# Jiawei-Yang/Denoising-ViT

Measured on AMD Instinct MI355X. Metric: stage-1 images denoised/sec (DINOv2-B/14, 518px, 1k Adam steps), higher is better.
Workload: dtype bf16

## Files before the change

denoising-vit_amd/csrc/dvt_fit_fused.hip:

```cpp
#include "dvt_common.h"
#include "dvt_grid_dev.h"
#include "dvt_loss_row.h"

typedef short bf16x8 __attribute__((ext_vector_type(8)));
typedef float f32x4 __attribute__((ext_vector_type(4)));

int g_fit_rows32 = 1;
int g_fit_xcd_affinity = 1;
int g_fit_small_wg = 0;

namespace {

constexpr int FR0 = 16;
constexpr int FW8 = 8;
constexpr int FE = 128;

template <bool F32>
struct Op {
  static constexpr int ES = F32 ? 4 : 2;
  static constexpr int KS = F32 ? 16 : 32;
};
typedef unsigned u32x4f __attribute__((ext_vector_type(4)));

template <bool F32>
__host__ __device__ constexpr int apitch(int K) { return K * Op<F32>::ES + 16; }

struct FusedArgs {
  DvtGridTable T;
  DvtShadowLayout S;
  DvtTLayout TL;
  int n, lattice;
  int xcd_group;
  float grad_scale;
  long long off_grid, off_b1, off_b2, off_G, off_bh1, off_bh2, off_bh3;
  DvtFusedFit f[DVT_FIT_BATCH_MAX];
};

__device__ __forceinline__ uint16_t bf16_of(float v) { return (uint16_t)(dvt_pack_bf16x2(v, 0.f) & 0xffffu); }

template <int NC, int FR, int FW, bool F32>
__device__ __forceinline__ void store_T(const char* img, void* __restrict__ dstTv, int B, int b0, int tid) {
  constexpr int RPP = F32 ? 4 : 8;
  for (int item = tid; item < NC * (FR / RPP); item += 64 * FW) {
    const int grp = item / NC, col = item - grp * NC;
    const int brow = b0 + grp * RPP;
    const char* src = img + grp * RPP * apitch<F32>(NC) + col * Op<F32>::ES;
    if constexpr (F32) {
      const int sg = brow >> 4, g = (brow >> 2) & 3;
      float4 v;
      v.x = *reinterpret_cast<const float*>(src);
      v.y = *reinterpret_cast<const float*>(src + apitch<F32>(NC));
      v.z = *reinterpret_cast<const float*>(src + 2 * apitch<F32>(NC));
      v.w = *reinterpret_cast<const float*>(src + 3 * apitch<F32>(NC));
      const long long off = ((long long)(col >> 4) * (B >> 4) + sg) * 256 + (((g << 4) + (col & 15)) << 2);
      *reinterpret_cast<float4*>(static_cast<float*>(dstTv) + off) = v;
    } else {
      const int kstep = brow >> 5, g = (brow >> 3) & 3;
      uint32_t w[4];
#pragma unroll
      for (int j = 0; j < 4; ++j) {
        const uint32_t lo = *reinterpret_cast<const uint16_t*>(src + (2 * j) * apitch<F32>(NC));
        const uint32_t hi = *reinterpret_cast<const uint16_t*>(src + (2 * j + 1) * apitch<F32>(NC));
        w[j] = lo | (hi << 16);
      }
      const long long off = ((long long)(col >> 4) * (B >> 5) + kstep) * 512 + (((g << 4) + (col & 15)) << 3);
      *reinterpret_cast<uint4*>(static_cast<uint16_t*>(dstTv) + off) = make_uint4(w[0], w[1], w[2], w[3]);
    }
  }
}

template <int K, int N, bool RELU, bool MASK, int RB, int FW, bool F32>
__device__ __forceinline__ void mlp_layer(const char* actA, const void* __restrict__ Wv,
                                          const float* __restrict__ bias, char* act_out,
                                          float* __restrict__ gout, const char* mask, int wave, int lane) {
  constexpr int KS = Op<F32>::KS, ES = Op<F32>::ES;
  constexpr int NTILES = N / 16, NT = (NTILES + FW - 1) / FW, S = K / KS;
  constexpr int INFL = FW == 8 ? 24 : 16;
  constexpr int PD0 = INFL / NT > 16 ? 16 : (INFL / NT < 1 ? 1 : INFL / NT);
  constexpr int PD = PD0 < S ? PD0 : S;
  static_assert(K % KS == 0 && N % 16 == 0, "layer shape");
  const int lc = lane & 15, g = lane >> 4;
  f32x4 acc[RB][NT];
  const char* wp[NT];
#pragma unroll
  for (int i = 0; i < NT; ++i) {
#pragma unroll
    for (int rb = 0; rb < RB; ++rb) acc[rb][i] = (f32x4){0.f, 0.f, 0.f, 0.f};
    const int t = wave + FW * i;
    const int tt = (NTILES % FW == 0 || t < NTILES) ? t : 0;
    wp[i] = static_cast<const char*>(Wv) + (size_t)tt * S * 1024 + lane * 16;
  }
  u32x4f b[PD][NT];
#pragma unroll
  for (int p = 0; p < PD; ++p)
#pragma unroll
    for (int i = 0; i < NT; ++i) b[p][i] = *reinterpret_cast<const u32x4f*>(wp[i] + 1024 * p);
  __builtin_amdgcn_sched_barrier(0);
  const char* ap = actA + lc * apitch<F32>(K) + g * 16;
#pragma unroll
  for (int s = 0; s < S; ++s) {
    u32x4f av[RB];
#pragma unroll
    for (int rb = 0; rb < RB; ++rb) av[rb] = *reinterpret_cast<const u32x4f*>(ap + rb * 16 * apitch<F32>(K) + s * 64);
    if constexpr (F32) {
#pragma unroll
      for (int j = 0; j < 4; ++j)
#pragma unroll
        for (int i = 0; i < NT; ++i)
#pragma unroll
          for (int rb = 0; rb < RB; ++rb)
            acc[rb][i] = __builtin_amdgcn_mfma_f32_16x16x4f32(__uint_as_float(av[rb][j]), __uint_as_float(b[s % PD][i][j]),
                                                              acc[rb][i], 0, 0, 0);
    } else {
#pragma unroll
      for (int i = 0; i < NT; ++i)
#pragma unroll
        for (int rb = 0; rb < RB; ++rb)
          acc[rb][i] = __builtin_amdgcn_mfma_f32_16x16x32_bf16(__builtin_bit_cast(bf16x8, av[rb]),
                                                               __builtin_bit_cast(bf16x8, b[s % PD][i]), acc[rb][i], 0, 0, 0);
    }
    if (s + PD < S) {
#pragma unroll
      for (int i = 0; i < NT; ++i) b[s % PD][i] = *reinterpret_cast<const u32x4f*>(wp[i] + 1024 * (s + PD));
    }
    __builtin_amdgcn_sched_barrier(0);
  }
#pragma unroll
  for (int i = 0; i < NT; ++i) {
    const int t = wave + FW * i;
    if (NTILES % FW != 0 && t >= NTILES) continue;
    const int n = t * 16 + lc;
    const float bv = bias != nullptr ? bias[n] : 0.f;
#pragma unroll
    for (int rb = 0; rb < RB; ++rb)
#pragma unroll
      for (int r = 0; r < 4; ++r) {
        const int row = rb * 16 + 4 * g + r;
        float v = acc[rb][i][r] + bv;
        if (RELU) v = fmaxf(v, 0.f);
        if (MASK) {
          if constexpr (F32) {
            v = *reinterpret_cast<const float*>(mask + row * apitch<F32>(N) + n * ES) > 0.f ? v : 0.f;
          } else {
            const uint16_t m = *reinterpret_cast<const uint16_t*>(mask + row * apitch<F32>(N) + n * ES);
            v = (m != 0 && !(m & 0x8000u)) ? v : 0.f;
          }
        }
        if (act_out != nullptr) {
          if constexpr (F32) *reinterpret_cast<float*>(act_out + row * apitch<F32>(N) + n * ES) = v;
          else *reinterpret_cast<uint16_t*>(act_out + row * apitch<F32>(N) + n * ES) = bf16_of(v);
        }
        if (gout != nullptr) gout[(size_t)row * N + n] = v;
      }
  }
}

template <int C, bool PH2, int FR, bool F32 = false>
struct FusedLds {
  static constexpr int H = C / 2, R = C / 4;
  static constexpr int O_ENC = 0;
  static constexpr int O_H1 = O_ENC + FR * apitch<F32>(FE);
  static constexpr int O_DF = O_H1 + FR * apitch<F32>(H);
  static constexpr int O_RAW = O_DF + FR * apitch<F32>(C);
  static constexpr int O_R1 = O_RAW + FR * apitch<F32>(C);
  static constexpr int O_R2 = O_R1 + FR * apitch<F32>(R);
  static constexpr int TOTAL = PH2 ? O_R2 + FR * apitch<F32>(R) : O_RAW;
};
template <int C>
constexpr bool fused_f32_fits() { return FusedLds<C, true, 16, true>::TOTAL <= 160 * 1024; }

template <int C, bool PH2, int FR, int FW, bool F32 = false>
__global__ __launch_bounds__(64 * FW) void fit_rows_kernel(FusedArgs a) {
  using L = FusedLds<C, PH2, FR, F32>;
  constexpr int RB = FR / 16;
  constexpr int ES = Op<F32>::ES;
  static_assert(FR == 16 || FR == 32, "rows per workgroup");
  static_assert(FW == 8 || (FW == 4 && FR == 16), "waves per workgroup");
  static_assert(!F32 || (FR == 16 && FW == 8), "fp32 operands: 16 rows, 8 waves");
  static_assert(L::TOTAL <= 160 * 1024, "LDS images of the row kernel");
  constexpr int H = C / 2, R = C / 4, E = FE, cq = C / 4;
  __shared__ __attribute__((aligned(16))) char smem[L::TOTAL];
  int fit_, rb_;
  if (a.xcd_group > 0) {
    const int lin = (int)blockIdx.x + (int)blockIdx.y * (int)gridDim.x, xcd = lin & 7, j = lin >> 3;
    fit_ = xcd / a.xcd_group;
    rb_ = j * a.xcd_group + xcd % a.xcd_group;
  } else {
    fit_ = (int)blockIdx.y;
    rb_ = (int)blockIdx.x;
  }
  const DvtFusedFit& f = a.f[fit_];
  const int tid = threadIdx.x, lane = tid & 63;
  const int wave = __builtin_amdgcn_readfirstlane(tid >> 6);
  const int row0 = rb_ * FR;
  const char* __restrict__ sh = static_cast<const char*>(f.shadow);
  const float* __restrict__ P = f.params;
  const float4* __restrict__ feat4 = reinterpret_cast<const float4*>(f.feat);

  uint32_t warm[5] = {0u, 0u, 0u, 0u, 0u};
  {
    constexpr int LPR = (C * 4 + 127) / 128;
    const int j = lane % 32;
#pragma unroll
    for (int rr = lane / 32; rr < FR / FW; rr += 2) {
      if (j < LPR) {
        const int ri = f.ridx[row0 + wave + FW * rr];
        warm[4] ^= __float_as_uint(f.feat[(size_t)ri * C + j * 32]) ^
                   __float_as_uint(P[a.off_G + (size_t)(ri % a.lattice) * C + j * 32]);
      }
    }
  }
  {
    const int per_xcd = a.xcd_group > 0 ? (int)gridDim.x / a.xcd_group : ((int)gridDim.x + 7) / 8;
    const int nslot = per_xcd >= 16 ? 16 : per_xcd;
    const int slot = (a.xcd_group > 0 ? rb_ / a.xcd_group : (rb_ >> 3)) % nslot;
    const long long lines = ((PH2 ? a.S.total : a.S.direct[2]) * ES + 127) / 128;
    const long long per = (lines + nslot - 1) / nslot;
    const long long l0 = slot * per, l1 = l0 + per < lines ? l0 + per : lines;
    const uint32_t* w32 = reinterpret_cast<const uint32_t*>(sh);
#pragma unroll
    for (int j = 0; j < 4 * RB * (8 / FW); ++j) {
      const long long li = l0 + tid + (long long)j * 64 * FW;
      if (li < l1) warm[j & 3] ^= w32[li * 32];
    }
  }

  if (tid < FR * 16) {
    const int r = tid >> 4, l = tid & 15;
    const float2 p = reinterpret_cast<const float2*>(f.xy)[f.ridx[row0 + r]];
    uint32_t idx[4];
    float w[4];
    corners2d(a.T, l, p.x, p.y, idx, w);
    const float4* __restrict__ grid = reinterpret_cast<const float4*>(P + a.off_grid);
    float4 lo = make_float4(0.f, 0.f, 0.f, 0.f), hi = lo;
#pragma unroll
    for (int c = 0; c < 4; ++c) {
      const float4 u = grid[(size_t)idx[c] * 2], v = grid[(size_t)idx[c] * 2 + 1];
      lo.x = fmaf(w[c], u.x, lo.x);
      lo.y = fmaf(w[c], u.y, lo.y);
      lo.z = fmaf(w[c], u.z, lo.z);
      lo.w = fmaf(w[c], u.w, lo.w);
      hi.x = fmaf(w[c], v.x, hi.x);
      hi.y = fmaf(w[c], v.y, hi.y);
      hi.z = fmaf(w[c], v.z, hi.z);
      hi.w = fmaf(w[c], v.w, hi.w);
    }
    if constexpr (F32) {
      *reinterpret_cast<float4*>(smem + L::O_ENC + r * apitch<F32>(E) + l * 32) = lo;
      *reinterpret_cast<float4*>(smem + L::O_ENC + r * apitch<F32>(E) + l * 32 + 16) = hi;
    } else {
      *reinterpret_cast<uint4*>(smem + L::O_ENC + r * apitch<F32>(E) + l * 16) =
          make_uint4(dvt_pack_bf16x2(lo.x, lo.y), dvt_pack_bf16x2(lo.z, lo.w), dvt_pack_bf16x2(hi.x, hi.y),
                     dvt_pack_bf16x2(hi.z, hi.w));
    }
  }
  if (PH2) {
    for (int i = tid; i < FR * cq; i += 64 * FW) {
      const int r = i / cq, q = i - r * cq;
      const float4 v = feat4[(size_t)f.ridx[row0 + r] * cq + q];
      if constexpr (F32)
        *reinterpret_cast<float4*>(smem + L::O_RAW + r * apitch<F32>(C) + q * 16) = v;
      else
        *reinterpret_cast<uint2*>(smem + L::O_RAW + r * apitch<F32>(C) + q * 8) =
            make_uint2(dvt_pack_bf16x2(v.x, v.y), dvt_pack_bf16x2(v.z, v.w));
    }
  }
  __syncthreads();

  const int B = a.n;
  char* __restrict__ T = static_cast<char*>(f.T);
#define SH(off) (sh + (size_t)(off) * ES)
#define TT(idx) (T + (size_t)a.TL.off[idx] * ES)
  mlp_layer<E, H, true, false, RB, FW, F32>(smem + L::O_ENC, SH(a.S.direct[0]), P + a.off_b1, smem + L::O_H1, nullptr,
                               nullptr, wave, lane);
  if (PH2)
    mlp_layer<C, R, true, false, RB, FW, F32>(smem + L::O_RAW, SH(a.S.direct[2]), P + a.off_bh1, smem + L::O_R1, nullptr,
                                 nullptr, wave, lane);
  __syncthreads();
  mlp_layer<H, C, false, false, RB, FW, F32>(smem + L::O_H1, SH(a.S.direct[1]), P + a.off_b2, nullptr,
                                f.F + (size_t)row0 * C, nullptr, wave, lane);
  store_T<H, FR, FW, F32>(smem + L::O_H1, TT(DVT_T_H1), B, row0, tid);
  store_T<E, FR, FW, F32>(smem + L::O_ENC, TT(DVT_T_ENC), B, row0, tid);
  if (PH2) {
    mlp_layer<R, R, true, false, RB, FW, F32>(smem + L::O_R1, SH(a.S.direct[3]), P + a.off_bh2, smem + L::O_R2, nullptr,
                                 nullptr, wave, lane);
    store_T<C, FR, FW, F32>(smem + L::O_RAW, TT(DVT_T_RAW), B, row0, tid);
    store_T<R, FR, FW, F32>(smem + L::O_R1, TT(DVT_T_R1), B, row0, tid);
    __syncthreads();
    mlp_layer<R, C, false, false, RB, FW, F32>(smem + L::O_R2, SH(a.S.direct[4]), P + a.off_bh3, nullptr,
                                  f.Hres + (size_t)row0 * C, nullptr, wave, lane);
    store_T<R, FR, FW, F32>(smem + L::O_R2, TT(DVT_T_R2), B, row0, tid);
  }
  __syncthreads();

  static_assert(C <= 1024, "row warm-up above assumes <= 32 lines per row");
  {
    constexpr int NR = FR / FW;
    constexpr int NB = (C <= 768 && !(FW == 4 && PH2)) ? 2 : 1;
    DvtLossRowRegs<PH2> lr[NB];
#pragma unroll
    for (int r0 = 0; r0 < NR; r0 += NB) {
#pragma unroll
    for (int rr = r0; rr < r0 + NB; ++rr) {
      const int gr = row0 + wave + FW * rr;
      const int ri = f.ridx[gr];
      dvt_loss_row_load<PH2>(lr[rr - r0], reinterpret_cast<const float4*>(f.F) + (size_t)gr * cq,
                             reinterpret_cast<const float4*>(P + a.off_G) + (size_t)(ri % a.lattice) * cq,
                             PH2 ? reinterpret_cast<const float4*>(f.Hres) + (size_t)gr * cq : nullptr,
                             feat4 + (size_t)ri * cq, cq, lane);
    }
#pragma unroll
    for (int rr = r0; rr < r0 + NB; ++rr) {
      const int row = wave + FW * rr, gr = row0 + row;
      char* const img_p = smem + L::O_DF + row * apitch<F32>(C);
      char* const img_h = PH2 ? smem + L::O_RAW + row * apitch<F32>(C) : nullptr;
      dvt_loss_row_compute<PH2>(lr[rr - r0], reinterpret_cast<float4*>(f.dF) + (size_t)gr * cq,
                                nullptr, nullptr,
                                f.rows + (size_t)gr * 8, a.n, cq, a.grad_scale, lane,
                                F32 ? nullptr : reinterpret_cast<uint2*>(img_p), F32 ? nullptr : reinterpret_cast<uint2*>(img_h),
                                F32 ? reinterpret_cast<float4*>(img_p) : nullptr, F32 ? reinterpret_cast<float4*>(img_h) : nullptr);
    }
    }
  }
  __syncthreads();

  mlp_layer<C, H, false, true, RB, FW, F32>(smem + L::O_DF, SH(a.S.transp[1]), nullptr, smem + L::O_H1, nullptr,
                               smem + L::O_H1, wave, lane);
  store_T<C, FR, FW, F32>(smem + L::O_DF, TT(DVT_T_DF), B, row0, tid);
  if (PH2) {
    mlp_layer<C, R, false, true, RB, FW, F32>(smem + L::O_RAW, SH(a.S.transp[4]), nullptr, smem + L::O_R2, nullptr,
                                 smem + L::O_R2, wave, lane);
    store_T<C, FR, FW, F32>(smem + L::O_RAW, TT(DVT_T_DH), B, row0, tid);
  }
  __syncthreads();
  mlp_layer<H, E, false, false, RB, FW, F32>(smem + L::O_H1, SH(a.S.transp[0]), nullptr, nullptr,
                                f.denc + (size_t)row0 * E, nullptr, wave, lane);
  store_T<H, FR, FW, F32>(smem + L::O_H1, TT(DVT_T_DH1), B, row0, tid);
  if (PH2) {
    mlp_layer<R, R, false, true, RB, FW, F32>(smem + L::O_R2, SH(a.S.transp[3]), nullptr, smem + L::O_R1, nullptr,
                                 smem + L::O_R1, wave, lane);
    store_T<R, FR, FW, F32>(smem + L::O_R2, TT(DVT_T_DR2), B, row0, tid);
    __syncthreads();
    store_T<R, FR, FW, F32>(smem + L::O_R1, TT(DVT_T_DR1), B, row0, tid);
  }
#undef SH
#undef TT
  if (a.n < 0) f.rows[tid] = __uint_as_float(warm[0] ^ warm[1] ^ warm[2] ^ warm[3] ^ warm[4]);
}

__global__ __launch_bounds__(256) void shadow_build_kernel(DvtShadowLayout L, const float* const p0,
                                                           const float* const p1, const float* const p2,
                                                           const float* const p3, void* s0, void* s1,
                                                           void* s2, void* s3, long long q_lo, long long q_hi) {
  const float* p = blockIdx.y == 0 ? p0 : (blockIdx.y == 1 ? p1 : (blockIdx.y == 2 ? p2 : p3));
  void* sh = blockIdx.y == 0 ? s0 : (blockIdx.y == 1 ? s1 : (blockIdx.y == 2 ? s2 : s3));
  const long long q = q_lo + (long long)blockIdx.x * 256 + threadIdx.x;
  if (q >= q_hi) return;
  dvt_shadow_store(L, sh, q * 4, reinterpret_cast<const float4*>(p)[q]);
}


constexpr int WG_MAX_PROB = 5 * DVT_FIT_BATCH_MAX;
struct WgradProb {
  const char* AT;
  const char* BT;
  float* dW;
  float* db;
  int M, N;
};
struct WgradGather {
  const int32_t* offs;
  const uint16_t* perm;
  const float4* rows;
  float4* dG;
};
struct WgradArgs {
  int n_prob, B, ksplit, units_total;
  int n_gather, lattice, cq;
  WgradGather gg[DVT_FIT_BATCH_MAX];
  int unit0[WG_MAX_PROB + 1];
  WgradProb p[WG_MAX_PROB];
};

constexpr int WG_PART_FLOATS = 32 * 32 + 32;
template <int SLOTS, bool F32>
__device__ __forceinline__ void wgrad_block(const WgradArgs& a, int blk, int wave, int lane, float* red) {
  constexpr int PD = 4;
  const int slot = wave >> 2, ks = wave & 3;
  const int unit = blk * SLOTS + slot;
  float* mine = red + (slot * 4 + ks) * WG_PART_FLOATS;
  const bool is_w = unit < a.units_total;
  const int gu = unit - a.units_total;
  float* out_w = nullptr;
  float* out_b = nullptr;
  int out_n = 0;
  int mb = 0, nb = 0;
  bool do_bias = false;
  if (is_w) {
    int pi = 0;
#pragma unroll
    for (int j = 1; j < WG_MAX_PROB; ++j)
      if (j < a.n_prob && unit >= a.unit0[j]) pi = j;
    const WgradProb& p = a.p[pi];
    out_w = p.dW;
    out_b = p.db;
    out_n = p.N;
    const int local = unit - a.unit0[pi], nbn = p.N >> 5;
    mb = local / nbn;
    nb = local - mb * nbn;
    const int ksteps = a.B / Op<F32>::KS, S = ksteps >> 2, s_begin = ks * S;
    const char* ap[2];
    const char* bp[2];
#pragma unroll
    for (int i = 0; i < 2; ++i) {
      ap[i] = p.AT + ((size_t)(mb * 2 + i) * ksteps + s_begin) * 1024 + lane * 16;
      bp[i] = p.BT + ((size_t)(nb * 2 + i) * ksteps + s_begin) * 1024 + lane * 16;
    }
    f32x4 acc[2][2];
#pragma unroll
    for (int i = 0; i < 2; ++i)
#pragma unroll
      for (int j = 0; j < 2; ++j) acc[i][j] = (f32x4){0.f, 0.f, 0.f, 0.f};
    do_bias = p.db != nullptr && nb == 0;
    float bsum[2] = {0.f, 0.f};
    u32x4f fa[PD][2], fb[PD][2];
#pragma unroll
    for (int q = 0; q < PD; ++q)
#pragma unroll
      for (int i = 0; i < 2; ++i) {
        fa[q][i] = *reinterpret_cast<const u32x4f*>(ap[i] + 1024 * q);
        fb[q][i] = *reinterpret_cast<const u32x4f*>(bp[i] + 1024 * q);
      }
    __builtin_amdgcn_sched_barrier(0);
    for (int s0 = 0; s0 < S; s0 += PD) {
#pragma unroll
      for (int q = 0; q < PD; ++q) {
        if constexpr (F32) {
#pragma unroll
          for (int e = 0; e < 4; ++e)
#pragma unroll
            for (int i = 0; i < 2; ++i)
#pragma unroll
              for (int j = 0; j < 2; ++j)
                acc[i][j] = __builtin_amdgcn_mfma_f32_16x16x4f32(__uint_as_float(fa[q][i][e]), __uint_as_float(fb[q][j][e]),
                                                                 acc[i][j], 0, 0, 0);
        } else {
#pragma unroll
          for (int i = 0; i < 2; ++i)
#pragma unroll
            for (int j = 0; j < 2; ++j)
              acc[i][j] = __builtin_amdgcn_mfma_f32_16x16x32_bf16(__builtin_bit_cast(bf16x8, fa[q][i]),
                                                                  __builtin_bit_cast(bf16x8, fb[q][j]), acc[i][j], 0, 0, 0);
        }
        if (do_bias) {
#pragma unroll
          for (int i = 0; i < 2; ++i) {
            if constexpr (F32) {
#pragma unroll
              for (int e = 0; e < 4; ++e) bsum[i] += __uint_as_float(fa[q][i][e]);
            } else {
#pragma unroll
              for (int e = 0; e < 4; ++e) {
                bsum[i] += __uint_as_float(fa[q][i][e] << 16);
                bsum[i] += __uint_as_float(fa[q][i][e] & 0xffff0000u);
              }
            }
          }
        }
        if (s0 + q + PD < S) {
#pragma unroll
          for (int i = 0; i < 2; ++i) {
            fa[q][i] = *reinterpret_cast<const u32x4f*>(ap[i] + 1024 * (s0 + q + PD));
            fb[q][i] = *reinterpret_cast<const u32x4f*>(bp[i] + 1024 * (s0 + q + PD));
          }
        }
        __builtin_amdgcn_sched_barrier(0);
      }
    }
#pragma unroll
    for (int i = 0; i < 2; ++i)
#pragma unroll
      for (int j = 0; j < 2; ++j)
#pragma unroll
        for (int r = 0; r < 4; ++r) mine[((i * 2 + j) * 4 + r) * 64 + lane] = acc[i][j][r];
    if (do_bias) {
#pragma unroll
      for (int i = 0; i < 2; ++i) {
        float v = bsum[i];
        v += __shfl_xor(v, 16, 64);
        v += __shfl_xor(v, 32, 64);
        if (lane < 16) mine[1024 + i * 16 + lane] = v;
      }
    }
  }
  __syncthreads();
  if (is_w) {
    if (ks != 0) return;
    const float* base = red + slot * 4 * WG_PART_FLOATS;
    const int lc = lane & 15, g = lane >> 4;
#pragma unroll
    for (int i = 0; i < 2; ++i)
#pragma unroll
      for (int j = 0; j < 2; ++j)
#pragma unroll
        for (int r = 0; r < 4; ++r) {
          const int o = ((i * 2 + j) * 4 + r) * 64 + lane;
          const float v = (base[o] + base[WG_PART_FLOATS + o]) + (base[2 * WG_PART_FLOATS + o] + base[3 * WG_PART_FLOATS + o]);
          out_w[(size_t)(mb * 32 + i * 16 + 4 * g + r) * out_n + nb * 32 + j * 16 + lc] = v;
        }
    if (do_bias && lane < 32) {
      const int o = 1024 + lane;
      out_b[mb * 32 + lane] = (base[o] + base[WG_PART_FLOATS + o]) + (base[2 * WG_PART_FLOATS + o] + base[3 * WG_PART_FLOATS + o]);
    }
    return;
  }
  const int u = gu * 4 + ks;
  if (u >= a.n_gather * a.lattice) return;
  const int fi = u / a.lattice, r = u - fi * a.lattice;
  const WgradGather& gg = a.gg[fi];
  const int o0 = gg.offs[r], o1 = gg.offs[r + 1];
  if (o1 == o0) return;
  for (int q = lane; q < a.cq; q += 64) {
    float4 acc4 = make_float4(0.f, 0.f, 0.f, 0.f);
    for (int o = o0; o < o1; ++o) {
      const float4 d = gg.rows[(size_t)gg.perm[o] * a.cq + q];
      acc4.x += d.x;
      acc4.y += d.y;
      acc4.z += d.z;
      acc4.w += d.w;
    }
    gg.dG[(size_t)r * a.cq + q] = acc4;
  }
}

struct BackwardArgs {
  DvtGridTable T;
  GridBwdPlan plan;
  GridBwdPtrs gp;
  GridSortedPtrs gs;
  int n, grid_blocks_per_fit, k, wg_blocks;
  WgradArgs w;
};
template <int WAVES, bool F32 = false>
__global__ __launch_bounds__(64 * WAVES) void fit_backward_kernel(BackwardArgs a) {
  __shared__ __attribute__((aligned(16))) float smem[WAVES * WG_PART_FLOATS];
  if ((int)blockIdx.x >= a.wg_blocks) {
    const int b = (int)blockIdx.x - a.wg_blocks;
    const int fy = b / a.grid_blocks_per_fit, bx = b - fy * a.grid_blocks_per_fit;
    if (a.gs.nt > 0) {
      const int parts = a.gs.nt / (64 * WAVES);
      grid_gather_body(a.T, a.gs, fy, bx / parts, bx % parts, a.gp.d_enc[fy], a.gp.d_params[fy], a.gp.touched[fy], 64 * WAVES);
      return;
    }
    if constexpr (WAVES == 16)
      grid_bwd_body<256>(a.T, a.plan, a.gp, a.n, bx, fy, smem, reinterpret_cast<uint32_t*>(smem + 256 * 8));
    return;
  }
  const int wave = __builtin_amdgcn_readfirstlane(threadIdx.x >> 6);
  wgrad_block<WAVES / 4, F32>(a.w, (int)blockIdx.x, wave, threadIdx.x & 63, smem);
}

template <int C>
int launch_rows(const FusedArgs& a, int k, bool phase2, hipStream_t s) {
  if (a.S.f32) {
    if constexpr (fused_f32_fits<C>()) {
      dim3 grid(a.n / 16, k), block(64 * FW8);
      if (phase2) hipLaunchKernelGGL((fit_rows_kernel<C, true, 16, FW8, true>), grid, block, 0, s, a);
      else hipLaunchKernelGGL((fit_rows_kernel<C, false, 16, FW8, true>), grid, block, 0, s, a);
      DVT_CHECK_LAUNCH();
      return 0;
    }
    return DVT_E_BADARG;
  }
  const bool fits32 = phase2 ? (FusedLds<C, true, 32>::TOTAL <= 160 * 1024) : (FusedLds<C, false, 32>::TOTAL <= 160 * 1024);
  const bool r32 = fits32 && a.n % 32 == 0 && (g_fit_rows32 == 2 || (g_fit_rows32 == 1 && k >= 4));
  const bool small = g_fit_small_wg && !r32;
  dim3 grid(a.n / (r32 ? 32 : 16), k), block(64 * (small ? 4 : FW8));
  FusedArgs ax = a;
  ax.xcd_group = (g_fit_xcd_affinity && (k == 2 || k == 4) && grid.x % (8 / k) == 0 && (grid.x * k) % 8 == 0) ? 8 / k : 0;
  const FusedArgs& a_ = ax;
  if (r32) {
    if (phase2) {
      if constexpr (FusedLds<C, true, 32>::TOTAL <= 160 * 1024) hipLaunchKernelGGL((fit_rows_kernel<C, true, 32, FW8>), grid, block, 0, s, a_);
    } else {
      if constexpr (FusedLds<C, false, 32>::TOTAL <= 160 * 1024) hipLaunchKernelGGL((fit_rows_kernel<C, false, 32, FW8>), grid, block, 0, s, a_);
    }
  } else if (small) {
    if (phase2) hipLaunchKernelGGL((fit_rows_kernel<C, true, 16, 4>), grid, block, 0, s, a_);
    else hipLaunchKernelGGL((fit_rows_kernel<C, false, 16, 4>), grid, block, 0, s, a_);
  } else if (phase2) {
    hipLaunchKernelGGL((fit_rows_kernel<C, true, 16, FW8>), grid, block, 0, s, a_);
  } else {
    hipLaunchKernelGGL((fit_rows_kernel<C, false, 16, FW8>), grid, block, 0, s, a_);
  }
  DVT_CHECK_LAUNCH();
  return 0;
}

}

int dvt_shadow_layout(const DvtFitConfig* c, DvtShadowLayout* L) {
  if (!c || !L) return DVT_E_BADARG;
  const int C = c->feat_dim, H = c->hidden, R = c->res_hidden;
  const int E = c->grid.n_levels * c->grid.n_features;
  const int Ns[DVT_SHADOW_MATS] = {H, C, R, R, C}, Ks[DVT_SHADOW_MATS] = {E, H, C, R, R};
  const long long begins[DVT_SHADOW_MATS] = {c->off_w1, c->off_w2, c->off_wh1, c->off_wh2, c->off_wh3};
  const bool tr[DVT_SHADOW_MATS] = {true, true, false, true, true};
  long long o = 0;
  L->n = DVT_SHADOW_MATS;
  L->f32 = c->mlp_bf16 ? 0 : 1;
  L->lo = begins[0];
  L->hi = 0;
  for (int i = 0; i < DVT_SHADOW_MATS; ++i) {
    if (Ks[i] % 32 || Ns[i] % 16 || (tr[i] && (Ns[i] % 32 || Ks[i] % 16))) return DVT_E_BADARG;
    L->N[i] = Ns[i];
    L->K[i] = Ks[i];
    L->begin[i] = begins[i];
    const long long sz = (long long)Ns[i] * Ks[i];
    L->direct[i] = o;
    o += sz;
    L->transp[i] = tr[i] ? o : -1;
    if (tr[i]) o += sz;
    if (begins[i] < L->lo) L->lo = begins[i];
    if (begins[i] + sz > L->hi) L->hi = begins[i] + sz;
  }
  L->total = o;
  return 0;
}

int dvt_shadow_build_k(const DvtShadowLayout* L, int k, const float* const* params, void* const* shadow,
                       long long lo, long long hi, hipStream_t s) {
  if (!L || k < 1 || k > DVT_FIT_BATCH_MAX || L->n <= 0) return DVT_E_BADARG;
  const float* p[4] = {nullptr, nullptr, nullptr, nullptr};
  void* sh[4] = {nullptr, nullptr, nullptr, nullptr};
  for (int f = 0; f < k; ++f) {
    if (!params[f] || !shadow[f]) return DVT_E_BADARG;
    p[f] = params[f];
    sh[f] = shadow[f];
  }
  const long long q_lo = (lo > L->lo ? lo : L->lo) / 4, q_hi = (hi < L->hi ? hi : L->hi) / 4;
  if (q_hi <= q_lo) return 0;
  hipLaunchKernelGGL(shadow_build_kernel, dim3(dvt_cdiv(q_hi - q_lo, 256), k), dim3(256), 0, s, *L, p[0], p[1],
                     p[2], p[3], sh[0], sh[1], sh[2], sh[3], q_lo, q_hi);
  DVT_CHECK_LAUNCH();
  return 0;
}

int g_fit_fused_enable = 1;
int g_fit_sorted_grid = 1;

int g_fit_fused_f32 = 1;

bool dvt_fit_fused_ok(const DvtFitConfig* c) {
  if (!g_fit_fused_enable || !c || !dvt_fit_fused_shapes_ok(c)) return false;
  if (c->mlp_bf16) return true;
  return g_fit_fused_f32 && (c->feat_dim == 384 || c->feat_dim == 768);
}

bool dvt_fit_fused_shapes_ok(const DvtFitConfig* c) {
  if (!c) return false;
  if (c->grid.n_levels != 16 || c->grid.n_features != 8) return false;
  const int C = c->feat_dim;
  if (C != 384 && C != 768 && C != 1024) return false;
  if (c->hidden != C / 2 || c->res_hidden != C / 4) return false;
  if (c->batch % 512 || c->batch <= 0) return false;
  return c->lattice <= 8192 && c->batch <= 65535;
}

int dvt_fit_rows_k(const DvtFitConfig* c, const DvtShadowLayout* L, int k, const DvtFusedFit* fits, bool phase2,
                   hipStream_t s) {
  if (!dvt_fit_fused_ok(c) || !L || !fits || k < 1 || k > DVT_FIT_BATCH_MAX) return DVT_E_BADARG;
  FusedArgs a{};
  a.T = c->grid;
  a.S = *L;
  dvt_t_layout(c, &a.TL);
  a.n = c->batch;
  a.lattice = c->lattice;
  a.grad_scale = (float)c->grad_scale;
  a.off_grid = c->off_grid;
  a.off_b1 = c->off_b1;
  a.off_b2 = c->off_b2;
  a.off_G = c->off_G;
  a.off_bh1 = c->off_bh1;
  a.off_bh2 = c->off_bh2;
  a.off_bh3 = c->off_bh3;
  for (int f = 0; f < k; ++f) a.f[f] = fits[f];
  const double C = c->feat_dim, H = c->hidden, R = c->res_hidden, E = FE, B = c->batch;
  const double flops = 2.0 * B * (2.0 * (E * H + H * C) + (phase2 ? (C * R + 2.0 * R * R + 2.0 * R * C) : 0.0));
  DvtProbeScope probe(DVT_PROBE_FIT_ROWS, s, flops * k);
  switch (c->feat_dim) {
    case 384: return launch_rows<384>(a, k, phase2, s);
    case 768: return launch_rows<768>(a, k, phase2, s);
    default: return launch_rows<1024>(a, k, phase2, s);
  }
}

void dvt_t_layout(const DvtFitConfig* c, DvtTLayout* L) {
  const int C = c->feat_dim, H = c->hidden, R = c->res_hidden, E = c->grid.n_levels * c->grid.n_features;
  const int cols[DVT_T_COUNT] = {C, H, H, E, C, R, R, C, R, R};
  long long o = 0;
  for (int i = 0; i < DVT_T_COUNT; ++i) {
    L->off[i] = o;
    L->cols[i] = cols[i];
    o += (long long)cols[i] * c->batch;
  }
  L->total = o;
}

int dvt_fit_backward_k(const DvtFitConfig* c, int k, const DvtFusedFit* fits, bool phase2, hipStream_t s) {
  if (!dvt_fit_fused_ok(c) || !fits || k < 1 || k > DVT_FIT_BATCH_MAX) return DVT_E_BADARG;
  DvtTLayout TL;
  dvt_t_layout(c, &TL);
  const int C = c->feat_dim, H = c->hidden, R = c->res_hidden, E = c->grid.n_levels * c->grid.n_features;
  BackwardArgs ba{};
  WgradArgs& a = ba.w;
  a.B = c->batch;
  const int ksteps = a.B / 32;
  a.ksplit = 4;
  if (ksteps % 16) return DVT_E_BADARG;
  int units = 0;
  double flops = 0.0;
  const bool f32 = !c->mlp_bf16;
  const size_t es = f32 ? 4 : 2;
  auto add = [&](const DvtFusedFit& f, int tA, int tB, long long ow, long long ob, int M, int N) {
    WgradProb& p = a.p[a.n_prob];
    p.AT = static_cast<const char*>(f.T) + (size_t)TL.off[tA] * es;
    p.BT = static_cast<const char*>(f.T) + (size_t)TL.off[tB] * es;
    p.dW = f.grads + ow;
    p.db = f.grads + ob;
    p.M = M;
    p.N = N;
    a.unit0[a.n_prob++] = units;
    units += (M / 32) * (N / 32);
    flops += 2.0 * M * N * a.B;
  };
  for (int f = 0; f < k; ++f) {
    add(fits[f], DVT_T_DF, DVT_T_H1, c->off_w2, c->off_b2, C, H);
    add(fits[f], DVT_T_DH1, DVT_T_ENC, c->off_w1, c->off_b1, H, E);
    if (phase2) {
      add(fits[f], DVT_T_DH, DVT_T_R2, c->off_wh3, c->off_bh3, C, R);
      add(fits[f], DVT_T_DR2, DVT_T_R1, c->off_wh2, c->off_bh2, R, R);
      add(fits[f], DVT_T_DR1, DVT_T_RAW, c->off_wh1, c->off_bh1, R, C);
    }
  }
  a.unit0[a.n_prob] = units;
  a.units_total = units;
  a.lattice = c->lattice;
  a.cq = C / 4;
  if (!phase2) {
    for (int f = 0; f < k; ++f) {
      if (!fits[f].g_offs || !fits[f].g_perm) return DVT_E_BADARG;
      a.gg[f] = WgradGather{fits[f].g_offs, fits[f].g_perm, reinterpret_cast<const float4*>(fits[f].dF),
                            reinterpret_cast<float4*>(fits[f].grads + c->off_G)};
    }
    a.n_gather = k;
  }
  ba.T = c->grid;
  ba.n = c->batch;
  ba.k = k;
  const int saved_chunk = g_grid_lds_chunk;
  g_grid_lds_chunk = 256;
  dvt_grid_bwd_plan(c->grid, c->batch, &ba.plan);
  g_grid_lds_chunk = saved_chunk;
  const long long direct_threads = (long long)c->batch * (c->grid.n_levels - ba.plan.first_direct_level) * 8;
  ba.grid_blocks_per_fit = ba.plan.n_lds_blocks + dvt_cdiv(direct_threads, 1024);
  bool sorted = g_fit_sorted_grid && dvt_grid_sorted_ok(&c->grid, c->batch);
  for (int f = 0; f < k; ++f) sorted = sorted && fits[f].gs_keys && fits[f].gs_pay && fits[f].gs_w;
  const bool small = g_fit_small_wg && sorted && !f32;
  if (sorted) {
    ba.gs.nt = 4 * c->batch;
    ba.gs.bitmap_end = fits[0].gs_bitmap_end;
    ba.grid_blocks_per_fit = c->grid.n_levels * (ba.gs.nt / (small ? 512 : 1024));
    for (int f = 0; f < k; ++f) {
      ba.gs.keys[f] = fits[f].gs_keys;
      ba.gs.pay[f] = fits[f].gs_pay;
      ba.gs.w[f] = fits[f].gs_w;
    }
  }
  for (int f = 0; f < k; ++f) {
    ba.gp.xy[f] = reinterpret_cast<const float2*>(fits[f].xy);
    ba.gp.ridx[f] = fits[f].ridx;
    ba.gp.d_enc[f] = fits[f].denc;
    ba.gp.d_params[f] = fits[f].grads + c->off_grid;
    ba.gp.touched[f] = fits[f].touched;
  }
  const int wg_blocks = dvt_cdiv((long long)units + dvt_cdiv((long long)a.n_gather * a.lattice, 4), small ? 2 : 4);
  ba.wg_blocks = wg_blocks;
  DvtProbeScope probe(DVT_PROBE_FIT_GEMM, s, flops);
  if (f32)
    hipLaunchKernelGGL((fit_backward_kernel<16, true>), dim3(ba.grid_blocks_per_fit * k + wg_blocks), dim3(1024), 0, s, ba);
  else if (small)
    hipLaunchKernelGGL(fit_backward_kernel<8>, dim3(ba.grid_blocks_per_fit * k + wg_blocks), dim3(512), 0, s, ba);
  else
    hipLaunchKernelGGL(fit_backward_kernel<16>, dim3(ba.grid_blocks_per_fit * k + wg_blocks), dim3(1024), 0, s, ba);
  DVT_CHECK_LAUNCH();
  return 0;
}
```

denoising-vit_amd/csrc/dvt_gemm_f32.hip:

```cpp
#include "dvt_common.h"

typedef float floatx16 __attribute__((ext_vector_type(16)));

namespace {

constexpr int BK = 64;
constexpr int LDK = BK + 4;

struct GemmArgs {
  const float* A;
  const float* B;
  float* C;
  int M, N, K;
  int lda, ldb, ldc;
  const float* bias;
  const float* mask;
  int ldmask;
  float* colsum;
  int relu;
  int kchunk;
  int atomic;
  int epi;
  const float* gamma;
  const float* smul;
  const float* rowsub;
  float oscale;
};

template <bool KCONTIG, int R, int NT, int BK>
struct Tile {
  static constexpr int LDK = BK + 4;
  static constexpr int NF4 = R * BK / 4;
  static constexpr int ITERS = (NF4 + NT - 1) / NT;
  static constexpr int LDS_FLOATS = KCONTIG ? R * LDK : BK * R;

  __device__ static __forceinline__ void load(const float* __restrict__ X, int ld, int r0, int Rmax,
                                              int k0, int kend, int tid, float4 regs[ITERS]) {
#pragma unroll
    for (int i = 0; i < ITERS; ++i) {
      const int f = tid + NT * i;
      float4 v = make_float4(0.f, 0.f, 0.f, 0.f);
      if (NF4 % NT == 0 || f < NF4) {
        if (KCONTIG) {
          const int r = f / (BK / 4), kq = f % (BK / 4);
          const int gr = r0 + r, gk = k0 + 4 * kq;
          if (gr < Rmax && gk < kend) v = *reinterpret_cast<const float4*>(X + (size_t)gr * ld + gk);
        } else {
          const int k = f / (R / 4), rq = f % (R / 4);
          const int gk = k0 + k, gr = r0 + 4 * rq;
          if (gk < kend && gr < Rmax) v = *reinterpret_cast<const float4*>(X + (size_t)gk * ld + gr);
        }
      }
      regs[i] = v;
    }
  }

  __device__ static __forceinline__ void store(float* __restrict__ S, int tid,
                                               const float4 regs[ITERS]) {
#pragma unroll
    for (int i = 0; i < ITERS; ++i) {
      const int f = tid + NT * i;
      if (NF4 % NT == 0 || f < NF4) {
        if (KCONTIG) {
          const int r = f / (BK / 4), kq = f % (BK / 4);
          *reinterpret_cast<float4*>(S + r * LDK + 4 * kq) = regs[i];
        } else {
          const int k = f / (R / 4), rq = f % (R / 4);
          *reinterpret_cast<float4*>(S + k * R + 4 * rq) = regs[i];
        }
      }
    }
  }

  __device__ static __forceinline__ void frags(const float* __restrict__ S, int row, int kh,
                                               float (&f)[BK / 2]) {
    if (KCONTIG) {
      const float4* p = reinterpret_cast<const float4*>(S + row * LDK + kh * (BK / 2));
#pragma unroll
      for (int q = 0; q < BK / 8; ++q) {
        const float4 v = p[q];
        f[4 * q + 0] = v.x;
        f[4 * q + 1] = v.y;
        f[4 * q + 2] = v.z;
        f[4 * q + 3] = v.w;
      }
    } else {
#pragma unroll
      for (int kk = 0; kk < BK / 2; ++kk) f[kk] = S[(kh * (BK / 2) + kk) * R + row];
    }
  }
};

template <bool A_KC, bool B_KC, int WM, int WN, int BK>
__device__ __forceinline__ void gemm_f32_body(const GemmArgs& p, int bx, int by, int bz,
                                              float* __restrict__ As, float* __restrict__ Bs) {
  constexpr int NT = 64 * WM * WN, BM = 32 * WM, BN = 32 * WN;
  using TA = Tile<A_KC, BM, NT, BK>;
  using TB = Tile<B_KC, BN, NT, BK>;
  const int tid = threadIdx.x;
  const int lane = tid & 63, wave = tid >> 6;
  const int wm = wave / WN, wn = wave % WN;
  const int n0 = bx * BN, m0 = by * BM;
  const int kbeg = bz * p.kchunk;
  const int kend = min(p.K, kbeg + p.kchunk);
  if (kbeg >= kend) return;

  floatx16 acc;
#pragma unroll
  for (int i = 0; i < 16; ++i) acc[i] = 0.f;
  float csum = 0.f;
  const bool do_colsum = (!A_KC) && p.colsum != nullptr && bx == 0;

  float4 ra[TA::ITERS], rb[TB::ITERS];
  TA::load(p.A, p.lda, m0, p.M, kbeg, kend, tid, ra);
  TB::load(p.B, p.ldb, n0, p.N, kbeg, kend, tid, rb);
  for (int k0 = kbeg; k0 < kend; k0 += BK) {
    TA::store(As, tid, ra);
    TB::store(Bs, tid, rb);
    __syncthreads();
    if (k0 + BK < kend) {
      TA::load(p.A, p.lda, m0, p.M, k0 + BK, kend, tid, ra);
      TB::load(p.B, p.ldb, n0, p.N, k0 + BK, kend, tid, rb);
    }
    const int ar = wm * 32 + (lane & 31), bc = wn * 32 + (lane & 31), kh = lane >> 5;
    float fa[BK / 2], fb[BK / 2];
    TA::frags(As, ar, kh, fa);
    TB::frags(Bs, bc, kh, fb);
#pragma unroll
    for (int kk = 0; kk < BK / 2; ++kk)
      acc = __builtin_amdgcn_mfma_f32_32x32x2f32(fa[kk], fb[kk], acc, 0, 0, 0);
    if (do_colsum && tid < BM) {
#pragma unroll 8
      for (int k = 0; k < BK; ++k) csum += As[k * BM + tid];
    }
    __syncthreads();
  }

  const int gn = n0 + wn * 32 + (lane & 31);
  const float bias = (p.bias != nullptr && gn < p.N) ? p.bias[gn] : 0.f;
#pragma unroll
  for (int r = 0; r < 16; ++r) {
    const int row = (r & 3) + 8 * (r >> 2) + 4 * (lane >> 5);
    const int gm = m0 + wm * 32 + row;
    if (gm < p.M && gn < p.N) {
      float v = acc[r] + bias;
      if (p.relu) v = fmaxf(v, 0.f);
      if (p.mask != nullptr) v = p.mask[(size_t)gm * p.ldmask + gn] > 0.f ? v : 0.f;
      if (p.smul != nullptr) v = p.oscale * p.smul[(size_t)gm * p.ldc + gn] * (v - p.rowsub[gm]);
      float* c = p.C + (size_t)gm * p.ldc + gn;
      if (p.atomic)
        atomic_add_f32(c, v);
      else
        *c = v;
    }
  }
  if (do_colsum && tid < BM && m0 + tid < p.M) atomic_add_f32(p.colsum + m0 + tid, csum);
}

template <bool A_KC, bool B_KC, int WM, int WN, int BK>
__global__ __launch_bounds__(64 * WM * WN) void gemm_f32_kernel(GemmArgs p) {
  constexpr int NT = 64 * WM * WN;
  __shared__ __attribute__((aligned(16))) float As[Tile<A_KC, 32 * WM, NT, BK>::LDS_FLOATS];
  __shared__ __attribute__((aligned(16))) float Bs[Tile<B_KC, 32 * WN, NT, BK>::LDS_FLOATS];
  gemm_f32_body<A_KC, B_KC, WM, WN, BK>(p, blockIdx.x, blockIdx.y, blockIdx.z, As, Bs);
}

constexpr int MULTI_MAX = 16;
struct MultiArgs {
  int n;
  int blk0[MULTI_MAX + 1];
  int gx[MULTI_MAX], gy[MULTI_MAX];
  int layout[MULTI_MAX];
  GemmArgs g[MULTI_MAX];
};

template <int BK>
__global__ __launch_bounds__(256) void gemm_f32_multi_kernel(MultiArgs m) {
  __shared__ __attribute__((aligned(16))) float As[64 * (BK + 4)];
  __shared__ __attribute__((aligned(16))) float Bs[64 * (BK + 4)];
  int i = 0;
#pragma unroll
  for (int j = 1; j < MULTI_MAX; ++j)
    if (j < m.n && (int)blockIdx.x >= m.blk0[j]) i = j;
  const int local = (int)blockIdx.x - m.blk0[i];
  const int bx = local % m.gx[i], by = (local / m.gx[i]) % m.gy[i], bz = local / (m.gx[i] * m.gy[i]);
  switch (m.layout[i]) {
    case 0: gemm_f32_body<true, true, 2, 2, BK>(m.g[i], bx, by, bz, As, Bs); break;
    case 1: gemm_f32_body<true, false, 2, 2, BK>(m.g[i], bx, by, bz, As, Bs); break;
    default: gemm_f32_body<false, false, 2, 2, BK>(m.g[i], bx, by, bz, As, Bs); break;
  }
}

typedef short bf16x8_t __attribute__((ext_vector_type(8)));
typedef float f32x2_t __attribute__((ext_vector_type(2)));
typedef __bf16 hwbf16x2_t __attribute__((ext_vector_type(2)));
__device__ __forceinline__ uint32_t pack_bf16x2(float a, float b) {
  const hwbf16x2_t v = __builtin_convertvector((f32x2_t){a, b}, hwbf16x2_t);
  return __builtin_bit_cast(uint32_t, v);
}


template <bool KCONTIG, int HBK>
struct TileH {
  static constexpr int HP = HBK + 8;
  static constexpr int ITERS = HBK / 16;
  __device__ static __forceinline__ void load(const float* __restrict__ X, int ld, int r0, int Rmax,
                                              int k0, int kend, int tid, float4 regs[ITERS]) {
#pragma unroll
    for (int i = 0; i < ITERS; ++i) {
      float4 v = make_float4(0.f, 0.f, 0.f, 0.f);
      if (KCONTIG) {
        const int f = tid + 256 * i, r = f / (HBK / 4), kq = f % (HBK / 4);
        const int gr = r0 + r, gk = k0 + 4 * kq;
        if (gr < Rmax && gk < kend) v = *reinterpret_cast<const float4*>(X + (size_t)gr * ld + gk);
      } else {
        const int kp = (tid >> 4) + 16 * (i >> 1), rq = tid & 15;
        const int gk = k0 + 2 * kp + (i & 1), gr = r0 + 4 * rq;
        if (gk < kend && gr < Rmax) v = *reinterpret_cast<const float4*>(X + (size_t)gk * ld + gr);
      }
      regs[i] = v;
    }
  }
  __device__ static __forceinline__ void store(uint16_t* __restrict__ S, int tid, const float4 regs[ITERS]) {
    if (KCONTIG) {
#pragma unroll
      for (int i = 0; i < ITERS; ++i) {
        const int f = tid + 256 * i, r = f / (HBK / 4), kq = f % (HBK / 4);
        uint2 w;
        w.x = pack_bf16x2(regs[i].x, regs[i].y);
        w.y = pack_bf16x2(regs[i].z, regs[i].w);
        *reinterpret_cast<uint2*>(S + r * HP + 4 * kq) = w;
      }
    } else {
      const int rq = tid & 15;
      uint32_t* S32 = reinterpret_cast<uint32_t*>(S);
#pragma unroll
      for (int it = 0; it < ITERS / 2; ++it) {
        const int kp = (tid >> 4) + 16 * it;
        const float4 lo = regs[2 * it], hi = regs[2 * it + 1];
        S32[((4 * rq + 0) * HP >> 1) + kp] = pack_bf16x2(lo.x, hi.x);
        S32[((4 * rq + 1) * HP >> 1) + kp] = pack_bf16x2(lo.y, hi.y);
        S32[((4 * rq + 2) * HP >> 1) + kp] = pack_bf16x2(lo.z, hi.z);
        S32[((4 * rq + 3) * HP >> 1) + kp] = pack_bf16x2(lo.w, hi.w);
      }
    }
  }
};

template <bool A_KC, bool B_KC, int HBK>
__device__ __forceinline__ void gemm_bf16op_body(const GemmArgs& p, int bx, int by, int bz,
                                                 uint16_t* __restrict__ As, uint16_t* __restrict__ Bs) {
  using TA = TileH<A_KC, HBK>;
  using TB = TileH<B_KC, HBK>;
  constexpr int HP = TA::HP, NR = TA::ITERS;
  const int tid = threadIdx.x;
  const int lane = tid & 63, wave = tid >> 6;
  const int wm = wave >> 1, wn = wave & 1;
  const int n0 = bx * 64, m0 = by * 64;
  const int kbeg = bz * p.kchunk;
  const int kend = min(p.K, kbeg + p.kchunk);
  if (kbeg >= kend) return;

  floatx16 acc;
#pragma unroll
  for (int i = 0; i < 16; ++i) acc[i] = 0.f;
  float csum = 0.f;
  const bool do_colsum = (!A_KC) && p.colsum != nullptr && bx == 0;

  float4 ra0[NR], rb0[NR], ra1[NR], rb1[NR];
  TA::load(p.A, p.lda, m0, p.M, kbeg, kend, tid, ra0);
  TB::load(p.B, p.ldb, n0, p.N, kbeg, kend, tid, rb0);
  TA::load(p.A, p.lda, m0, p.M, kbeg + HBK, kend, tid, ra1);
  TB::load(p.B, p.ldb, n0, p.N, kbeg + HBK, kend, tid, rb1);
  const int gn = n0 + wn * 32 + (lane & 31);
  const float bias = (p.bias != nullptr && gn < p.N) ? p.bias[gn] : 0.f;
  float mk[16];
#pragma unroll
  for (int r = 0; r < 16; ++r) {
    const int gm = m0 + wm * 32 + (r & 3) + 8 * (r >> 2) + 4 * (lane >> 5);
    mk[r] = (p.mask != nullptr && gm < p.M && gn < p.N) ? p.mask[(size_t)gm * p.ldmask + gn] : 1.f;
  }
  const int kh = lane >> 5;
  const uint16_t* pa = As + (wm * 32 + (lane & 31)) * HP + kh * (HBK / 2);
  const uint16_t* pb = Bs + (wn * 32 + (lane & 31)) * HP + kh * (HBK / 2);
#define H_STEP(RA, RB, KNEXT)                                                                  \
  do {                                                                                         \
    TA::store(As, tid, RA);                                                                    \
    TB::store(Bs, tid, RB);                                                                    \
    __syncthreads();                                                                           \
    TA::load(p.A, p.lda, m0, p.M, (KNEXT), kend, tid, RA);                \
    TB::load(p.B, p.ldb, n0, p.N, (KNEXT), kend, tid, RB);                                     \
    bf16x8_t fa[HBK / 16], fb[HBK / 16];                                                       \
    _Pragma("unroll") for (int q = 0; q < HBK / 16; ++q) {                                     \
      fa[q] = *reinterpret_cast<const bf16x8_t*>(pa + 8 * q);                                  \
      fb[q] = *reinterpret_cast<const bf16x8_t*>(pb + 8 * q);                                  \
    }                                                                                          \
    _Pragma("unroll") for (int q = 0; q < HBK / 16; ++q)                                       \
        acc = __builtin_amdgcn_mfma_f32_32x32x16_bf16(fa[q], fb[q], acc, 0, 0, 0);             \
    if (do_colsum && tid < 64) {  \
      const uint32_t* row = reinterpret_cast<const uint32_t*>(As + tid * HP);                  \
      _Pragma("unroll") for (int k = 0; k < HBK / 2; ++k) {                                    \
        const uint32_t w = row[k];                                                             \
        csum += __uint_as_float(w << 16) + __uint_as_float(w & 0xffff0000u);                   \
      }                                                                                        \
    }                                                                                          \
    __syncthreads();                                                                           \
  } while (0)
  for (int k0 = kbeg; k0 < kend; k0 += 2 * HBK) {
    H_STEP(ra0, rb0, k0 + 2 * HBK);
    if (k0 + HBK < kend) H_STEP(ra1, rb1, k0 + 3 * HBK);
  }
#undef H_STEP

#pragma unroll
  for (int r = 0; r < 16; ++r) {
    const int row = (r & 3) + 8 * (r >> 2) + 4 * (lane >> 5);
    const int gm = m0 + wm * 32 + row;
    if (gm < p.M && gn < p.N) {
      float v = acc[r] + bias;
      if (p.relu) v = fmaxf(v, 0.f);
      v = mk[r] > 0.f ? v : 0.f;
      float* c = p.C + (size_t)gm * p.ldc + gn;
      if (p.atomic)
        atomic_add_f32(c, v);
      else
        *c = v;
    }
  }
  if (do_colsum && tid < 64 && m0 + tid < p.M) atomic_add_f32(p.colsum + m0 + tid, csum);
}

template <int HBK>
__global__ __launch_bounds__(256) void gemm_bf16op_multi_kernel(MultiArgs m) {
  __shared__ __attribute__((aligned(16))) uint16_t As[64 * (HBK + 8)];
  __shared__ __attribute__((aligned(16))) uint16_t Bs[64 * (HBK + 8)];
  int i = 0;
#pragma unroll
  for (int j = 1; j < MULTI_MAX; ++j)
    if (j < m.n && (int)blockIdx.x >= m.blk0[j]) i = j;
  const int local = (int)blockIdx.x - m.blk0[i];
  const int bx = local % m.gx[i], by = (local / m.gx[i]) % m.gy[i], bz = local / (m.gx[i] * m.gy[i]);
  switch (m.layout[i]) {
    case 0: gemm_bf16op_body<true, true, HBK>(m.g[i], bx, by, bz, As, Bs); break;
    case 1: gemm_bf16op_body<true, false, HBK>(m.g[i], bx, by, bz, As, Bs); break;
    default: gemm_bf16op_body<false, false, HBK>(m.g[i], bx, by, bz, As, Bs); break;
  }
}

constexpr int G3_STAGE_FLOATS = 2 * 64 * BK;

__device__ __forceinline__ void glds16f(const void* gsrc, void* lds_wave_base) {
  __builtin_amdgcn_global_load_lds((const __attribute__((address_space(1))) void*)gsrc,
                                   (__attribute__((address_space(3))) void*)lds_wave_base, 16, 0, 0);
}

template <bool KCONTIG>
__device__ __forceinline__ void stage_f32(const float* __restrict__ X, int ld, int r0, int Rmax,
                                          int k0, float* lds, int wave, int lane) {
#pragma unroll
  for (int it = 0; it < 4; ++it) {
    const int s = it * 256 + wave * 64 + lane;
    const float* src;
    if (KCONTIG) {
      const int row = s >> 4, cp = s & 15, c = cp ^ (row & 15);
      src = X + (size_t)min(r0 + row, Rmax - 1) * ld + k0 + c * 4;
    } else {
      const int k = s >> 4, cq = s & 15;
      src = X + (size_t)(k0 + k) * ld + r0 + cq * 4;
    }
    glds16f(src, lds + (it * 256 + wave * 64) * 4);
  }
}

template <bool KCONTIG>
__device__ __forceinline__ void frags_f32(const float* __restrict__ S, int row, int kh,
                                          float (&f)[BK / 2]) {
  if (KCONTIG) {
#pragma unroll
    for (int q = 0; q < BK / 8; ++q) {
      const int chunk = (kh * (BK / 8) + q) ^ (row & 15);
      const float4 v = *reinterpret_cast<const float4*>(S + row * BK + chunk * 4);
      f[4 * q + 0] = v.x;
      f[4 * q + 1] = v.y;
      f[4 * q + 2] = v.z;
      f[4 * q + 3] = v.w;
    }
  } else {
#pragma unroll
    for (int kk = 0; kk < BK / 2; ++kk) f[kk] = S[(kh * (BK / 2) + kk) * 64 + row];
  }
}

template <bool A_KC, bool B_KC, int NS = 3>
__device__ __forceinline__ void gemm_f32_glds_body(const GemmArgs& p, int bz, float* __restrict__ smem) {
  const int tid = threadIdx.x, lane = tid & 63, wave = tid >> 6;
  const int wm = wave >> 1, wn = wave & 1;
  const int n0 = blockIdx.x * 64, m0 = blockIdx.y * 64;
  const int kbeg = bz * p.kchunk;
  const int kend = min(p.K, kbeg + p.kchunk);
  if (kbeg >= kend) return;
  const int nk = (kend - kbeg) / BK;

  floatx16 acc;
#pragma unroll
  for (int i = 0; i < 16; ++i) acc[i] = 0.f;
  float csum = 0.f;
  const bool do_colsum = (!A_KC) && p.colsum != nullptr && blockIdx.x == 0;

#define G3_ISSUE(kt)                                                                          \
  do {                                                                                        \
    float* st_ = smem + ((kt) % NS) * G3_STAGE_FLOATS;                                        \
    stage_f32<A_KC>(p.A, p.lda, m0, p.M, kbeg + (kt) * BK, st_, wave, lane);                  \
    stage_f32<B_KC>(p.B, p.ldb, n0, p.N, kbeg + (kt) * BK, st_ + 64 * BK, wave, lane);        \
  } while (0)
  G3_ISSUE(0);
  if (NS == 3 && nk > 1) G3_ISSUE(1);
  for (int kt = 0; kt < nk; ++kt) {
    if (NS == 3 && kt + 1 < nk)
      asm volatile("s_waitcnt vmcnt(8)" ::: "memory");
    else
      asm volatile("s_waitcnt vmcnt(0)" ::: "memory");
    __builtin_amdgcn_s_barrier();
    __builtin_amdgcn_sched_barrier(0);
    if (kt + NS - 1 < nk) G3_ISSUE(kt + NS - 1);
    const float* As = smem + (kt % NS) * G3_STAGE_FLOATS;
    const float* Bs = As + 64 * BK;
    const int ar = wm * 32 + (lane & 31), bc = wn * 32 + (lane & 31), kh = lane >> 5;
    float fa[BK / 2], fb[BK / 2];
    frags_f32<A_KC>(As, ar, kh, fa);
    frags_f32<B_KC>(Bs, bc, kh, fb);
#pragma unroll
    for (int kk = 0; kk < BK / 2; ++kk)
      acc = __builtin_amdgcn_mfma_f32_32x32x2f32(fa[kk], fb[kk], acc, 0, 0, 0);
    if (do_colsum && tid < 64) {
#pragma unroll 8
      for (int k = 0; k < BK; ++k) csum += As[k * 64 + tid];
    }
  }
#undef G3_ISSUE

  const int gn = n0 + wn * 32 + (lane & 31);
  const float bias = (p.bias != nullptr && gn < p.N) ? p.bias[gn] : 0.f;
#pragma unroll
  for (int r = 0; r < 16; ++r) {
    const int row = (r & 3) + 8 * (r >> 2) + 4 * (lane >> 5);
    const int gm = m0 + wm * 32 + row;
    if (gm < p.M && gn < p.N) {
      float v = acc[r] + bias;
      if (p.relu) v = fmaxf(v, 0.f);
      if (p.mask != nullptr) v = p.mask[(size_t)gm * p.ldmask + gn] > 0.f ? v : 0.f;
      float* c = p.C + (size_t)gm * p.ldc + gn;
      if (p.atomic)
        atomic_add_f32(c, v);
      else
        *c = v;
    }
  }
  if (do_colsum && tid < 64 && m0 + tid < p.M) atomic_add_f32(p.colsum + m0 + tid, csum);
}

template <bool A_KC, bool B_KC, int NS = 3>
__global__ __launch_bounds__(256) void gemm_f32_glds_kernel(GemmArgs p) {
  __shared__ __attribute__((aligned(16))) float smem[NS * G3_STAGE_FLOATS];
  gemm_f32_glds_body<A_KC, B_KC, NS>(p, blockIdx.z, smem);
}

struct BatchDims {
  int nb1;
  long long sA0, sA1, sB0, sB1, sC0, sC1;
};
template <bool A_KC, bool B_KC, int NS = 3>
__global__ __launch_bounds__(256) void gemm_f32_glds_batched_kernel(GemmArgs p, BatchDims d) {
  __shared__ __attribute__((aligned(16))) float smem[NS * G3_STAGE_FLOATS];
  const int b0 = blockIdx.z / d.nb1, b1 = blockIdx.z - b0 * d.nb1;
  GemmArgs q = p;
  q.A = p.A + b0 * d.sA0 + b1 * d.sA1;
  q.B = p.B + b0 * d.sB0 + b1 * d.sB1;
  q.C = p.C + b0 * d.sC0 + b1 * d.sC1;
  gemm_f32_glds_body<A_KC, B_KC, NS>(q, 0, smem);
}

template <bool A_KC, bool B_KC>
__global__ __launch_bounds__(256) void gemm_f32_batched_small_k_kernel(GemmArgs p, BatchDims d) {
  __shared__ __attribute__((aligned(16))) float As[Tile<A_KC, 64, 256, 64>::LDS_FLOATS];
  __shared__ __attribute__((aligned(16))) float Bs[Tile<B_KC, 64, 256, 64>::LDS_FLOATS];
  const int b0 = blockIdx.z / d.nb1, b1 = blockIdx.z - b0 * d.nb1;
  GemmArgs q = p;
  q.A = p.A + b0 * d.sA0 + b1 * d.sA1;
  q.B = p.B + b0 * d.sB0 + b1 * d.sB1;
  q.C = p.C + b0 * d.sC0 + b1 * d.sC1;
  if (p.smul != nullptr) {
    q.smul = p.smul + b0 * d.sC0 + b1 * d.sC1;
    q.rowsub = p.rowsub + (size_t)blockIdx.z * p.M;
  }
  gemm_f32_body<A_KC, B_KC, 2, 2, 64>(q, blockIdx.x, blockIdx.y, 0, As, Bs);
}

constexpr int GB_BK = 32;
constexpr int GB_TILE_FLOATS = 128 * GB_BK;
constexpr int GB_STAGE_FLOATS = 2 * GB_TILE_FLOATS;

__device__ __forceinline__ void stage_big(const float* __restrict__ X, int ld, int r0, int k0, float* lds, int wave, int lane) {
#pragma unroll
  for (int it = 0; it < 4; ++it) {
    const int s = it * 256 + wave * 64 + lane;
    const int row = s >> 3, c = (s & 7) ^ ((row >> 1) & 7);
    glds16f(X + (size_t)(r0 + row) * ld + k0 + c * 4, lds + (it * 256 + wave * 64) * 4);
  }
}

__device__ __forceinline__ float4 frag4_big(const float* __restrict__ S, int row, int kh, int q) {
  return *reinterpret_cast<const float4*>(S + row * GB_BK + (((kh * (GB_BK / 8) + q) ^ ((row >> 1) & 7)) << 2));
}

template <int EPI>
__global__ __launch_bounds__(256) void gemm_f32_big_kernel(GemmArgs p) {
  __shared__ __attribute__((aligned(16))) float smem[2 * GB_STAGE_FLOATS];
  const int tid = threadIdx.x, lane = tid & 63;
  const int wave = __builtin_amdgcn_readfirstlane(tid >> 6);
  const int wm = wave >> 1, wn = wave & 1;
  const int n0 = blockIdx.x * 128, m0 = blockIdx.y * 128;
  const int nk = p.K / GB_BK;
  floatx16 acc[2][2];
#pragma unroll
  for (int i = 0; i < 2; ++i)
#pragma unroll
    for (int j = 0; j < 2; ++j)
#pragma unroll
      for (int e = 0; e < 16; ++e) acc[i][j][e] = 0.f;
#define GB_ISSUE(kt)                                                             \
  do {                                                                           \
    float* st_ = smem + ((kt) & 1) * GB_STAGE_FLOATS;                            \
    stage_big(p.A, p.lda, m0, (kt) * GB_BK, st_, wave, lane);                    \
    stage_big(p.B, p.ldb, n0, (kt) * GB_BK, st_ + GB_TILE_FLOATS, wave, lane);   \
  } while (0)
  GB_ISSUE(0);
  const int l31 = lane & 31, kh = lane >> 5;
  for (int kt = 0; kt < nk; ++kt) {
    asm volatile("s_waitcnt vmcnt(0)" ::: "memory");
    __builtin_amdgcn_s_barrier();
    __builtin_amdgcn_sched_barrier(0);
    if (kt + 1 < nk) GB_ISSUE(kt + 1);
    const float* As = smem + (kt & 1) * GB_STAGE_FLOATS;
    const float* Bs = As + GB_TILE_FLOATS;
    float4 fa[2][GB_BK / 8], fb[2][GB_BK / 8];
#pragma unroll
    for (int q = 0; q < GB_BK / 8; ++q)
#pragma unroll
      for (int i = 0; i < 2; ++i) {
        fa[i][q] = frag4_big(As, wm * 64 + i * 32 + l31, kh, q);
        fb[i][q] = frag4_big(Bs, wn * 64 + i * 32 + l31, kh, q);
      }
#pragma unroll
    for (int q = 0; q < GB_BK / 8; ++q) {
#define GB_STEP(E)                                                                                          \
  _Pragma("unroll") for (int i = 0; i < 2; ++i)                                                             \
  _Pragma("unroll") for (int j = 0; j < 2; ++j)                                                             \
      acc[i][j] = __builtin_amdgcn_mfma_f32_32x32x2f32(fa[i][q].E, fb[j][q].E, acc[i][j], 0, 0, 0);
      GB_STEP(x) GB_STEP(y) GB_STEP(z) GB_STEP(w)
#undef GB_STEP
    }
  }
#undef GB_ISSUE
#pragma unroll
  for (int j = 0; j < 2; ++j) {
    const int gn = n0 + wn * 64 + j * 32 + l31;
    const float bias = p.bias != nullptr ? p.bias[gn] : 0.f;
    const float gm_n = EPI == 2 ? p.gamma[gn] : 0.f;
#pragma unroll
    for (int i = 0; i < 2; ++i)
#pragma unroll
      for (int r = 0; r < 16; ++r) {
        const int gm = m0 + wm * 64 + i * 32 + (r & 3) + 8 * (r >> 2) + 4 * kh;
        float v = acc[i][j][r] + bias;
        float* c = p.C + (size_t)gm * p.ldc + gn;
        if constexpr (EPI == 1) {
          v = 0.5f * v * (1.0f + erff(v * 0.70710678118654752f));
        } else if constexpr (EPI == 2) {
          v = *c + gm_n * v;
        } else {
          if (p.relu) v = fmaxf(v, 0.f);
        }
        *c = v;
      }
  }
}

__device__ __forceinline__ void stage_rows_big(const float* __restrict__ X, int ld, int k0, int c0, float* lds, int wave, int lane) {
#pragma unroll
  for (int it = 0; it < 4; ++it) {
    const int s = it * 256 + wave * 64 + lane;
    glds16f(X + (size_t)(k0 + (s >> 5)) * ld + c0 + (s & 31) * 4, lds + (it * 256 + wave * 64) * 4);
  }
}

__global__ __launch_bounds__(256) void gemm_f32_big_tn_kernel(GemmArgs p) {
  __shared__ __attribute__((aligned(16))) float smem[2 * GB_STAGE_FLOATS];
  const int tid = threadIdx.x, lane = tid & 63;
  const int wave = __builtin_amdgcn_readfirstlane(tid >> 6);
  const int wm = wave >> 1, wn = wave & 1;
  const int n0 = blockIdx.x * 128, m0 = blockIdx.y * 128;
  const int kbeg = blockIdx.z * p.kchunk, kend = kbeg + p.kchunk < p.K ? kbeg + p.kchunk : p.K;
  const int nk = (kend - kbeg) / GB_BK;
  const bool do_colsum = p.colsum != nullptr && blockIdx.x == 0 && wn == 0;
  floatx16 acc[2][2];
#pragma unroll
  for (int i = 0; i < 2; ++i)
#pragma unroll
    for (int j = 0; j < 2; ++j)
#pragma unroll
      for (int e = 0; e < 16; ++e) acc[i][j][e] = 0.f;
  float csum[2] = {0.f, 0.f};
#define GT_ISSUE(kt)                                                                       \
  do {                                                                                     \
    float* st_ = smem + ((kt) & 1) * GB_STAGE_FLOATS;                                      \
    stage_rows_big(p.A, p.lda, kbeg + (kt) * GB_BK, m0, st_, wave, lane);                  \
    stage_rows_big(p.B, p.ldb, kbeg + (kt) * GB_BK, n0, st_ + GB_TILE_FLOATS, wave, lane); \
  } while (0)
  if (nk > 0) GT_ISSUE(0);
  const int l31 = lane & 31, kh = lane >> 5;
  for (int kt = 0; kt < nk; ++kt) {
    asm volatile("s_waitcnt vmcnt(0)" ::: "memory");
    __builtin_amdgcn_s_barrier();
    __builtin_amdgcn_sched_barrier(0);
    if (kt + 1 < nk) GT_ISSUE(kt + 1);
    const float* As = smem + (kt & 1) * GB_STAGE_FLOATS + kh * 128 + wm * 64 + l31;
    const float* Bs = smem + (kt & 1) * GB_STAGE_FLOATS + GB_TILE_FLOATS + kh * 128 + wn * 64 + l31;
#pragma unroll
    for (int s = 0; s < GB_BK / 2; ++s) {
      const float a0 = As[s * 256], a1 = As[s * 256 + 32], b0 = Bs[s * 256], b1 = Bs[s * 256 + 32];
      acc[0][0] = __builtin_amdgcn_mfma_f32_32x32x2f32(a0, b0, acc[0][0], 0, 0, 0);
      acc[0][1] = __builtin_amdgcn_mfma_f32_32x32x2f32(a0, b1, acc[0][1], 0, 0, 0);
      acc[1][0] = __builtin_amdgcn_mfma_f32_32x32x2f32(a1, b0, acc[1][0], 0, 0, 0);
      acc[1][1] = __builtin_amdgcn_mfma_f32_32x32x2f32(a1, b1, acc[1][1], 0, 0, 0);
      if (do_colsum) {
        csum[0] += a0;
        csum[1] += a1;
      }
    }
  }
#undef GT_ISSUE
#pragma unroll
  for (int j = 0; j < 2; ++j) {
    const int gn = n0 + wn * 64 + j * 32 + l31;
#pragma unroll
    for (int i = 0; i < 2; ++i)
#pragma unroll
      for (int r = 0; r < 16; ++r) {
        const int gm = m0 + wm * 64 + i * 32 + (r & 3) + 8 * (r >> 2) + 4 * kh;
        float* c = p.C + (size_t)gm * p.ldc + gn;
        if (p.atomic)
          atomic_add_f32(c, acc[i][j][r]);
        else
          *c = acc[i][j][r];
      }
  }
  if (do_colsum) {
#pragma unroll
    for (int i = 0; i < 2; ++i) {
      const float v = csum[i] + __shfl_xor(csum[i], 32, 64);
      if (kh == 0) atomic_add_f32(p.colsum + m0 + wm * 64 + i * 32 + l31, v);
    }
  }
}

int g_f32_big = 1;
int g_f32_glds = 1;
int g_f32_ex_stages = 2;
extern int g_cfg_override;

template <bool A_KC, bool B_KC>
bool glds_ok(const GemmArgs& a) {
  if (!g_f32_glds || (a.K % BK) || (a.kchunk % BK) || g_cfg_override > 0) return false;
  if (!A_KC && (a.M % 64)) return false;
  if (!B_KC && (a.N % 64)) return false;
  return a.M >= 1 && a.N >= 1;
}

int g_cfg_override = -1;

struct TileCfg {
  int bm, bn;
};
constexpr TileCfg kCfgs[4] = {{64, 64}, {32, 64}, {32, 32}, {64, 32}};

int pick_cfg(int M, int N, int ksplits) {
  if (g_cfg_override >= 0 && g_cfg_override < 4) return g_cfg_override;
  (void)ksplits;
  if (M <= 32 || N <= 32) return 2;
  return 0;
}

int g_f32_bk = 32;

template <bool A_KC, bool B_KC, int WM, int WN, int BKT>
int launch_cfg(const GemmArgs& a, int ksplits, hipStream_t s) {
  dim3 grid(dvt_cdiv(a.N, 32 * WN), dvt_cdiv(a.M, 32 * WM), ksplits);
  DvtProbeScope probe(DVT_PROBE_FIT_GEMM, s, 2.0 * a.M * a.N * a.K);
  hipLaunchKernelGGL((gemm_f32_kernel<A_KC, B_KC, WM, WN, BKT>), grid, dim3(64 * WM * WN), 0, s, a);
  DVT_CHECK_LAUNCH();
  return 0;
}

template <bool A_KC, bool B_KC>
int launch(const GemmArgs& a, int ksplits, hipStream_t s) {
  if (g_f32_bk == 64 && glds_ok<A_KC, B_KC>(a)) {
    dim3 grid(dvt_cdiv(a.N, 64), dvt_cdiv(a.M, 64), ksplits);
    DvtProbeScope probe(DVT_PROBE_FIT_GEMM, s, 2.0 * a.M * a.N * a.K);
    hipLaunchKernelGGL((gemm_f32_glds_kernel<A_KC, B_KC>), grid, dim3(256), 0, s, a);
    DVT_CHECK_LAUNCH();
    return 0;
  }
  const int cfg = pick_cfg(a.M, a.N, ksplits);
  if (g_f32_bk == 16) return launch_cfg<A_KC, B_KC, 2, 2, 16>(a, ksplits, s);
  if (g_f32_bk == 32) return launch_cfg<A_KC, B_KC, 2, 2, 32>(a, ksplits, s);
  switch (cfg) {
    case 0: return launch_cfg<A_KC, B_KC, 2, 2, 64>(a, ksplits, s);
    case 1: return launch_cfg<A_KC, B_KC, 1, 2, 64>(a, ksplits, s);
    case 3: return launch_cfg<A_KC, B_KC, 2, 1, 64>(a, ksplits, s);
    default: return launch_cfg<A_KC, B_KC, 1, 1, 64>(a, ksplits, s);
  }
}

GemmArgs make_fwd(const float* x, const float* w, const float* b, float* y, int m, int n, int k,
                  int relu) {
  GemmArgs a{};
  a.A = x; a.B = w; a.C = y;
  a.M = m; a.N = n; a.K = k;
  a.lda = k; a.ldb = k; a.ldc = n;
  a.bias = b; a.relu = relu;
  a.kchunk = (k + 63) / 64 * 64;
  return a;
}

GemmArgs make_wgrad(const float* dy, const float* x, float* dw, float* db, int m, int n, int k,
                    int* splits_out) {
  GemmArgs a{};
  a.A = dy; a.B = x; a.C = dw;
  a.M = n; a.N = k; a.K = m;
  a.lda = n; a.ldb = k; a.ldc = k;
  a.colsum = db;
  a.atomic = 1;
  const int tiles = dvt_cdiv(n, 64) * dvt_cdiv(k, 64);
  const int ktiles = dvt_cdiv(m, 64);
  int splits = dvt_cdiv(384, tiles);
  if (splits > ktiles / 2) splits = ktiles / 2;
  if (splits < 1) splits = 1;
  a.kchunk = dvt_cdiv(ktiles, splits) * 64;
  *splits_out = dvt_cdiv(m, a.kchunk);
  return a;
}

GemmArgs make_dgrad(const float* dy, const float* w, float* dx, const float* relu_mask, int m,
                    int n, int k) {
  GemmArgs a{};
  a.A = dy; a.B = w; a.C = dx;
  a.M = m; a.N = k; a.K = n;
  a.lda = n; a.ldb = k; a.ldc = k;
  a.mask = relu_mask; a.ldmask = k;
  a.kchunk = (n + 63) / 64 * 64;
  return a;
}

}

int dvt_linear_group(const DvtLinearOp* ops, int n_ops, hipStream_t s, int bf16_operands) {
  if (!ops || n_ops < 1 || n_ops > MULTI_MAX) return DVT_E_BADARG;
  MultiArgs m{};
  m.n = n_ops;
  int blocks = 0;
  double flops = 0.0;
  for (int i = 0; i < n_ops; ++i) {
    const DvtLinearOp& o = ops[i];
    if (o.m <= 0 || o.n <= 0 || o.k <= 0 || (o.n & 3) || (o.k & 3)) return DVT_E_BADARG;
    int splits = 1;
    if (o.kind == 0) {
      m.g[i] = make_fwd(o.x, o.w, o.b, o.y, o.m, o.n, o.k, o.relu);
      m.layout[i] = 0;
    } else if (o.kind == 1) {
      m.g[i] = make_wgrad(o.dy, o.x, o.dw, o.db, o.m, o.n, o.k, &splits);
      m.layout[i] = 2;
    } else if (o.kind == 2) {
      m.g[i] = make_dgrad(o.dy, o.w, o.dx, o.relu_mask, o.m, o.n, o.k);
      m.layout[i] = 1;
    } else {
      return DVT_E_BADARG;
    }
    m.gx[i] = dvt_cdiv(m.g[i].N, 64);
    m.gy[i] = dvt_cdiv(m.g[i].M, 64);
    m.blk0[i] = blocks;
    blocks += m.gx[i] * m.gy[i] * splits;
    flops += 2.0 * o.m * o.n * o.k;
  }
  m.blk0[n_ops] = blocks;
  DvtProbeScope probe(DVT_PROBE_FIT_GEMM, s, flops);
  if (bf16_operands) {
    if (g_f32_bk == 64)
      hipLaunchKernelGGL(gemm_bf16op_multi_kernel<64>, dim3(blocks), dim3(256), 0, s, m);
    else
      hipLaunchKernelGGL(gemm_bf16op_multi_kernel<32>, dim3(blocks), dim3(256), 0, s, m);
  } else if (g_f32_bk == 16)
    hipLaunchKernelGGL(gemm_f32_multi_kernel<16>, dim3(blocks), dim3(256), 0, s, m);
  else if (g_f32_bk == 32)
    hipLaunchKernelGGL(gemm_f32_multi_kernel<32>, dim3(blocks), dim3(256), 0, s, m);
  else
    hipLaunchKernelGGL(gemm_f32_multi_kernel<64>, dim3(blocks), dim3(256), 0, s, m);
  DVT_CHECK_LAUNCH();
  return 0;
}

namespace {
extern int g_cfg_override;
}
extern int g_fit_fused_enable;
extern int g_fit_fused_f32;
extern int g_fit_sorted_grid;
extern int g_fit_lazy_adam;
extern int g_fit_lazy_refresh;
extern int g_fit_lazy_exact;
extern int g_fit_lazy_merge;
extern int g_fit_shadow_in_adam;
extern int g_adam_pingpong;
extern int g_fit_rows32;
extern int g_fit_small_wg;
extern int g_fit_xcd_affinity;
#ifdef DVT_LAB
extern int g_fit_skip_mask;
#endif

extern "C" int dvt_tune_set(int key, int value) {
  if (key == 0) {
    g_cfg_override = value;
    return 0;
  }
  if (key == 4) {
    if (value == 2 || value == 3)
      g_f32_ex_stages = value;
    else if (value == 10 || value == 11)
      g_f32_big = value == 11;
    else
      g_f32_glds = value;
    return 0;
  }
  if (key == 5) {
    if (value != 16 && value != 32 && value != 64) return DVT_E_BADARG;
    g_f32_bk = value;
    return 0;
  }
  if (key == 8) {
    g_adam_pingpong = value != 0;
    return 0;
  }
  if (key == 6) {
    if (value == 2 || value == 3)
      g_fit_fused_f32 = value == 3;
    else
      g_fit_fused_enable = value != 0;
    return 0;
  }
  if (key == 7) {
    g_fit_sorted_grid = value != 0;
    return 0;
  }
  if (key == 10) {
    g_fit_lazy_exact = value != 0;
    return 0;
  }
  if (key == 11) {
    g_fit_lazy_merge = value != 0;
    return 0;
  }
  if (key == 12) {
    g_fit_shadow_in_adam = value != 0;
    return 0;
  }
  if (key == 13) {
    if (value < 0 || value > 2) return DVT_E_BADARG;
    g_fit_rows32 = value;
    return 0;
  }
  if (key == 14) {
    g_fit_small_wg = value != 0;
    return 0;
  }
  if (key == 16) {
    g_fit_xcd_affinity = value != 0;
    return 0;
  }
#ifdef DVT_LAB
  if (key == 15) {
    g_fit_skip_mask = value & 7;
    return 0;
  }
#endif
  if (key == 9) {
    g_fit_lazy_adam = value != 0;
    if (value >= 2) g_fit_lazy_refresh = value;
    return 0;
  }
  if (key == 18) return dvt_s2_tune(value);
  if (key == 1) return dvt_vit_tune(value);
  if (key == 2) return dvt_grid_tune(value);
  if (key == 3) return dvt_adam_tune(value);
  return DVT_E_BADARG;
}

int dvt_gemm_f32_ex(const DvtGemmEx* g, hipStream_t s) {
  if (!g || !g->A || !g->B || !g->C || g->M <= 0 || g->N <= 0 || g->K <= 0) return DVT_E_BADARG;
  GemmArgs a{};
  a.A = g->A; a.B = g->B; a.C = g->C;
  a.M = g->M; a.N = g->N; a.K = g->K;
  a.lda = g->lda; a.ldb = g->ldb; a.ldc = g->ldc;
  a.bias = g->bias;
  a.colsum = g->layout == 2 ? g->colsum : nullptr;
  a.atomic = g->accumulate;
  if (g->smul != nullptr) {
    const int nb_ = (g->nb0 > 0 ? g->nb0 : 1) * (g->nb1 > 0 ? g->nb1 : 1);
    if (!g->rowsub || g->layout != 0 || nb_ <= 1 || g->K > BK || g->accumulate) return DVT_E_BADARG;
    a.smul = g->smul;
    a.rowsub = g->rowsub;
    a.oscale = g->oscale;
  }
  if (a.K % BK) return DVT_E_BADARG;
  const bool a_kc = g->layout != 2, b_kc = g->layout == 0;
  if ((!a_kc && (a.M % 64)) || (!b_kc && (a.N % 64)) || (a.lda & 3) || (a.ldb & 3)) return DVT_E_BADARG;
  const int nb = (g->nb0 > 0 ? g->nb0 : 1) * (g->nb1 > 0 ? g->nb1 : 1);
  int splits = 1;
  a.kchunk = a.K;
  if (g->accumulate && nb == 1) {
    const int tiles = dvt_cdiv(a.M, 64) * dvt_cdiv(a.N, 64), ktiles = a.K / BK;
    splits = dvt_cdiv(1024, tiles);
    if (splits > ktiles / 4) splits = ktiles / 4;
    if (splits < 1) splits = 1;
    a.kchunk = dvt_cdiv(ktiles, splits) * BK;
    splits = dvt_cdiv(a.K, a.kchunk);
  }
  if (nb > 65535 || splits > 65535) return DVT_E_BADARG;
  dim3 grid(dvt_cdiv(a.N, 64), dvt_cdiv(a.M, 64), nb > 1 ? nb : splits);
  DvtProbeScope probe(DVT_PROBE_FIT_GEMM, s, 2.0 * a.M * a.N * a.K * nb);
#define EX_LAUNCH(NS)                                                                                     \
  do {                                                                                                    \
    if (nb > 1) {                                                                                         \
      BatchDims d{g->nb1 > 0 ? g->nb1 : 1, g->sA0, g->sA1, g->sB0, g->sB1, g->sC0, g->sC1};               \
      if (a.K <= BK && g->layout == 0)                                                                    \
        hipLaunchKernelGGL((gemm_f32_batched_small_k_kernel<true, true>), grid, dim3(256), 0, s, a, d);   \
      else if (g->layout == 0)                                                                            \
        hipLaunchKernelGGL((gemm_f32_glds_batched_kernel<true, true, NS>), grid, dim3(256), 0, s, a, d);  \
      else if (g->layout == 1)                                                                            \
        hipLaunchKernelGGL((gemm_f32_glds_batched_kernel<true, false, NS>), grid, dim3(256), 0, s, a, d); \
      else                                                                                                \
        hipLaunchKernelGGL((gemm_f32_glds_batched_kernel<false, false, NS>), grid, dim3(256), 0, s, a, d);\
    } else {                                                                                              \
      if (g->layout == 0)                                                                                 \
        hipLaunchKernelGGL((gemm_f32_glds_kernel<true, true, NS>), grid, dim3(256), 0, s, a);             \
      else if (g->layout == 1)                                                                            \
        hipLaunchKernelGGL((gemm_f32_glds_kernel<true, false, NS>), grid, dim3(256), 0, s, a);            \
      else                                                                                                \
        hipLaunchKernelGGL((gemm_f32_glds_kernel<false, false, NS>), grid, dim3(256), 0, s, a);           \
    }                                                                                                     \
  } while (0)
  if (g_f32_ex_stages == 2)
    EX_LAUNCH(2);
  else
    EX_LAUNCH(3);
#undef EX_LAUNCH
  DVT_CHECK_LAUNCH();
  return 0;
}

bool dvt_linear_big_ok(int m, int n, int k) { return g_f32_big && m > 0 && m % 128 == 0 && n % 128 == 0 && k % GB_BK == 0; }

bool dvt_linear_wgrad_big_ok(int rows, int n, int k) { return g_f32_big && rows > 0 && rows % GB_BK == 0 && n % 128 == 0 && k % 128 == 0; }
int dvt_linear_wgrad_big(const float* dy, const float* x, float* dw, float* db, int rows, int n, int k, int accumulate,
                         hipStream_t s) {
  if (!dy || !x || !dw || !dvt_linear_wgrad_big_ok(rows, n, k)) return DVT_E_BADARG;
  GemmArgs a{};
  a.A = dy; a.B = x; a.C = dw;
  a.M = n; a.N = k; a.K = rows;
  a.lda = n; a.ldb = k; a.ldc = k;
  a.colsum = db;
  a.atomic = accumulate;
  const int tiles = (n / 128) * (k / 128), ktiles = rows / GB_BK;
  int splits = 1;
  if (accumulate) {
    splits = dvt_cdiv(1024, tiles);
    if (splits > ktiles / 8) splits = ktiles / 8;
    if (splits < 1) splits = 1;
  }
  a.kchunk = dvt_cdiv(ktiles, splits) * GB_BK;
  splits = dvt_cdiv(rows, a.kchunk);
  DvtProbeScope probe(DVT_PROBE_FIT_GEMM, s, 2.0 * a.M * a.N * a.K);
  hipLaunchKernelGGL(gemm_f32_big_tn_kernel, dim3(k / 128, n / 128, splits), dim3(256), 0, s, a);
  DVT_CHECK_LAUNCH();
  return 0;
}

int dvt_linear_fwd_big_epi(const float* x, const float* w, const float* b, float* y, int m, int n, int k, int epi,
                           const float* gamma, hipStream_t s) {
  if (!x || !w || !y || !dvt_linear_big_ok(m, n, k) || (epi != 1 && epi != 2) || (epi == 2 && !gamma)) return DVT_E_BADARG;
  GemmArgs a = make_fwd(x, w, b, y, m, n, k, 0);
  a.epi = epi;
  a.gamma = gamma;
  DvtProbeScope probe(DVT_PROBE_FIT_GEMM, s, 2.0 * a.M * a.N * a.K);
  if (epi == 1) hipLaunchKernelGGL(gemm_f32_big_kernel<1>, dim3(a.N / 128, a.M / 128), dim3(256), 0, s, a);
  else hipLaunchKernelGGL(gemm_f32_big_kernel<2>, dim3(a.N / 128, a.M / 128), dim3(256), 0, s, a);
  DVT_CHECK_LAUNCH();
  return 0;
}

int dvt_linear_fwd_big(const float* x, const float* w, const float* b, float* y, int m, int n, int k, hipStream_t s) {
  if (!x || !w || !y || m <= 0 || n <= 0 || k <= 0 || (k & 3) || (n & 3)) return DVT_E_BADARG;
  const GemmArgs a = make_fwd(x, w, b, y, m, n, k, 0);
  if (dvt_linear_big_ok(m, n, k)) {
    DvtProbeScope probe(DVT_PROBE_FIT_GEMM, s, 2.0 * a.M * a.N * a.K);
    hipLaunchKernelGGL(gemm_f32_big_kernel<0>, dim3(a.N / 128, a.M / 128), dim3(256), 0, s, a);
    DVT_CHECK_LAUNCH();
    return 0;
  }
  if ((a.K % BK) == 0 && (a.kchunk % BK) == 0) {
    dim3 grid(dvt_cdiv(a.N, 64), dvt_cdiv(a.M, 64), 1);
    DvtProbeScope probe(DVT_PROBE_FIT_GEMM, s, 2.0 * a.M * a.N * a.K);
    if (g_f32_ex_stages == 2)
      hipLaunchKernelGGL((gemm_f32_glds_kernel<true, true, 2>), grid, dim3(256), 0, s, a);
    else
      hipLaunchKernelGGL((gemm_f32_glds_kernel<true, true, 3>), grid, dim3(256), 0, s, a);
    DVT_CHECK_LAUNCH();
    return 0;
  }
  return launch<true, true>(a, 1, s);
}

extern "C" int dvt_linear_fwd(const float* x, const float* w, const float* b, float* y, int m,
                              int n, int k, int relu, void* stream) {
  if (!x || !w || !y || m < 0 || n <= 0 || k <= 0 || (k & 3) || (n & 3)) return DVT_E_BADARG;
  if (m == 0) return 0;
  return launch<true, true>(make_fwd(x, w, b, y, m, n, k, relu), 1, (hipStream_t)stream);
}

extern "C" int dvt_linear_bwd(const float* dy, const float* x, const float* w, float* dw,
                              float* db, float* dx, const float* relu_mask, int m, int n, int k,
                              void* stream) {
  if (!dy || m < 0 || n <= 0 || k <= 0 || (k & 3) || (n & 3)) return DVT_E_BADARG;
  if (m == 0) return 0;
  hipStream_t s = (hipStream_t)stream;
  if (dw != nullptr) {
    if (!x) return DVT_E_BADARG;
    int splits = 1;
    const GemmArgs a = make_wgrad(dy, x, dw, db, m, n, k, &splits);
    int rc = launch<false, false>(a, splits, s);
    if (rc) return rc;
  } else if (db != nullptr) {
    return DVT_E_BADARG;
  }
  if (dx != nullptr) {
    if (!w) return DVT_E_BADARG;
    int rc = launch<true, false>(make_dgrad(dy, w, dx, relu_mask, m, n, k), 1, s);
    if (rc) return rc;
  }
  return 0;
}
```

denoising-vit_amd/csrc/dvt_grid_dev.h:

```cpp
#pragma once
#include "dvt_common.h"

__device__ __forceinline__ void corners2d(const DvtGridTable& T, int l, float x, float y,
                                          uint32_t idx[4], float w[4]) {
  const float scale = T.scale[l];
  const uint32_t res = T.resolution[l];
  const uint32_t n = T.entries[l];
  const uint32_t off = T.offset[l];
  const bool hashed = T.hashed[l] != 0;
  const float px = fmaf(scale, x, 0.5f), py = fmaf(scale, y, 0.5f);
  const float fx = floorf(px), fy = floorf(py);
  const uint32_t cx = (uint32_t)(int)fx, cy = (uint32_t)(int)fy;
  const float wx = px - fx, wy = py - fy;
#pragma unroll
  for (int c = 0; c < 4; ++c) {
    const uint32_t ux = cx + (c & 1), uy = cy + ((c >> 1) & 1);
    uint32_t index = hashed ? (ux ^ (uy * 2654435761u)) : (ux + uy * res);
    index %= n;
    idx[c] = off + index;
    const float a = (c & 1) ? wx : 1.0f - wx;
    const float b = (c & 2) ? wy : 1.0f - wy;
    w[c] = a * b;
  }
}


struct GridBwdPlan {
  int n_lds_blocks;
  int first_direct_level;
  int chunk_start[DVT_MAX_LEVELS + 1];
  int splits[DVT_MAX_LEVELS];
};

struct GridBwdPtrs {
  const float2* xy[DVT_FIT_BATCH_MAX];
  const int32_t* ridx[DVT_FIT_BATCH_MAX];
  const float* d_enc[DVT_FIT_BATCH_MAX];
  float* d_params[DVT_FIT_BATCH_MAX];
  uint32_t* touched[DVT_FIT_BATCH_MAX];
  uint32_t bitmap_end;
};

template <int LDS_CHUNK>
__device__ __forceinline__ void grid_bwd_body(const DvtGridTable& T, const GridBwdPlan& plan, const GridBwdPtrs& q,
                                              int n, int bx, int fy, float* acc, uint32_t* flags) {
  const float2* __restrict__ xy = q.xy[fy];
  const int32_t* __restrict__ ridx = q.ridx[fy];
  const float* __restrict__ d_enc = q.d_enc[fy];
  float* __restrict__ d_params = q.d_params[fy];
  uint32_t* __restrict__ touched = q.touched[fy];
  const int L = T.n_levels;
  const int tid = threadIdx.x;
  if (bx < plan.n_lds_blocks) {
    int l = 0;
    while (l + 1 < plan.first_direct_level && bx >= plan.chunk_start[l + 1]) ++l;
    const int nsplit = plan.splits[l];
    const int local = bx - plan.chunk_start[l];
    const int split = local % nsplit;
    const uint32_t e0 = (uint32_t)(local / nsplit) * LDS_CHUNK;
    const int per = (n + nsplit - 1) / nsplit;
    const int b_begin = split * per, b_end = min(n, b_begin + per);
    const uint32_t abs0 = T.offset[l] + e0;
    const uint32_t cnt = min((uint32_t)LDS_CHUNK, T.entries[l] - e0);
    const uint32_t base32 = abs0 & ~31u;
    for (int i = tid; i < LDS_CHUNK * 8; i += 1024) acc[i] = 0.f;
    if (tid < LDS_CHUNK / 32 + 1) flags[tid] = 0u;
    __syncthreads();
    for (int b = b_begin + tid; b < b_end; b += 1024) {
      const float2 p = xy[ridx != nullptr ? ridx[b] : b];
      uint32_t idx[4];
      float w[4];
      corners2d(T, l, p.x, p.y, idx, w);
      bool any = false;
#pragma unroll
      for (int c = 0; c < 4; ++c) any |= (idx[c] - abs0) < cnt;
      if (!any) continue;
      const float4* gp = reinterpret_cast<const float4*>(d_enc + ((size_t)b * L + l) * 8);
      const float4 g0 = gp[0], g1 = gp[1];
#pragma unroll
      for (int c = 0; c < 4; ++c) {
        const uint32_t rel = idx[c] - abs0;
        if (rel < cnt) {
          float* a = acc + rel;
          atomicAdd(a + 0 * LDS_CHUNK, w[c] * g0.x);
          atomicAdd(a + 1 * LDS_CHUNK, w[c] * g0.y);
          atomicAdd(a + 2 * LDS_CHUNK, w[c] * g0.z);
          atomicAdd(a + 3 * LDS_CHUNK, w[c] * g0.w);
          atomicAdd(a + 4 * LDS_CHUNK, w[c] * g1.x);
          atomicAdd(a + 5 * LDS_CHUNK, w[c] * g1.y);
          atomicAdd(a + 6 * LDS_CHUNK, w[c] * g1.z);
          atomicAdd(a + 7 * LDS_CHUNK, w[c] * g1.w);
          atomicOr(&flags[(idx[c] - base32) >> 5], 1u << (idx[c] & 31u));
        }
      }
    }
    __syncthreads();
    for (uint32_t e = tid; e < cnt; e += 1024) {
      const uint32_t a = abs0 + e;
      if ((flags[(a - base32) >> 5] >> (a & 31u)) & 1u) {
        float4* dst = reinterpret_cast<float4*>(d_params + (size_t)a * 8);
        if (nsplit > 1) {
          float* d = d_params + (size_t)a * 8;
#pragma unroll
          for (int f = 0; f < 8; ++f) atomic_add_f32(d + f, acc[f * LDS_CHUNK + e]);
          continue;
        }
        const float4 o0 = dst[0], o1 = dst[1];
        const float4 s0 = make_float4(acc[e], acc[LDS_CHUNK + e], acc[2 * LDS_CHUNK + e],
                                      acc[3 * LDS_CHUNK + e]);
        const float4 s1 = make_float4(acc[4 * LDS_CHUNK + e], acc[5 * LDS_CHUNK + e],
                                      acc[6 * LDS_CHUNK + e], acc[7 * LDS_CHUNK + e]);
        dst[0] = make_float4(o0.x + s0.x, o0.y + s0.y, o0.z + s0.z, o0.w + s0.w);
        dst[1] = make_float4(o1.x + s1.x, o1.y + s1.y, o1.z + s1.z, o1.w + s1.w);
      }
    }
    if (touched != nullptr && tid < LDS_CHUNK / 32 + 1 && flags[tid] != 0u)
      __hip_atomic_fetch_or(touched + (base32 >> 5) + tid, flags[tid], __ATOMIC_RELAXED,
                            __HIP_MEMORY_SCOPE_AGENT);
    return;
  }
  const int nd = L - plan.first_direct_level;
  const long long t = (long long)(bx - plan.n_lds_blocks) * 1024 + tid;
  if (nd <= 0 || t >= (long long)n * nd * 8) return;
  const int f = (int)(t & 7);
  const long long bl = t >> 3;
  const int b = (int)(bl / nd), l = plan.first_direct_level + (int)(bl - (long long)b * nd);
  const float2 p = xy[ridx != nullptr ? ridx[b] : b];
  uint32_t idx[4];
  float w[4];
  corners2d(T, l, p.x, p.y, idx, w);
  const float g = d_enc[((size_t)b * L + l) * 8 + f];
#pragma unroll
  for (int c = 0; c < 4; ++c) {
    atomic_add_f32(d_params + (size_t)idx[c] * 8 + f, w[c] * g);
    if (touched != nullptr && f == 0 && (q.bitmap_end == 0u || idx[c] < q.bitmap_end)) {
      const uint32_t bit = 1u << (idx[c] & 31u);
      uint32_t* wp = touched + (idx[c] >> 5);
      if ((__hip_atomic_load(wp, __ATOMIC_RELAXED, __HIP_MEMORY_SCOPE_AGENT) & bit) == 0u)
        __hip_atomic_fetch_or(wp, bit, __ATOMIC_RELAXED, __HIP_MEMORY_SCOPE_AGENT);
    }
  }
}


struct GridSortedPtrs {
  const uint32_t* keys[DVT_FIT_BATCH_MAX];
  const uint16_t* pay[DVT_FIT_BATCH_MAX];
  const float* w[DVT_FIT_BATCH_MAX];
  int nt;
  uint32_t bitmap_end;
};

__device__ __forceinline__ void grid_gather_body(const DvtGridTable& T, const GridSortedPtrs& q, int fy, int l, int part,
                                                 const float* __restrict__ d_enc, float* __restrict__ d_params,
                                                 uint32_t* __restrict__ touched, int bs = 1024) {
  const int lane = threadIdx.x & 63;
  const int u = part * bs + threadIdx.x;
  const size_t base = (size_t)l * q.nt;
  const uint32_t* __restrict__ keys = q.keys[fy] + base;
  const uint32_t key = keys[u];
  const uint32_t prev = u > 0 ? keys[u - 1] : 0xffffffffu;
  const uint32_t next = u + 1 < q.nt ? keys[u + 1] : 0xffffffffu;
  const uint32_t pay = q.pay[fy][base + u];
  const float wgt = q.w[fy][base + u];
  const float4* gp = reinterpret_cast<const float4*>(d_enc + ((size_t)(pay >> 2) * T.n_levels + l) * 8);
  const float4 g0 = gp[0], g1 = gp[1];
  float c[8] = {wgt * g0.x, wgt * g0.y, wgt * g0.z, wgt * g0.w, wgt * g1.x, wgt * g1.y, wgt * g1.z, wgt * g1.w};
#pragma unroll
  for (int d = 1; d < 64; d <<= 1) {
    const uint32_t ok = __shfl_up(key, d, 64);
    const bool take = lane >= d && ok == key;
#pragma unroll
    for (int f = 0; f < 8; ++f) {
      const float o = __shfl_up(c[f], d, 64);
      if (take) c[f] += o;
    }
  }
  const uint32_t first_key = __builtin_amdgcn_readfirstlane(key), first_prev = __builtin_amdgcn_readfirstlane(prev);
  const bool ends = key != next;
  if (!(ends || lane == 63)) return;
  const bool began_before = key == first_key && first_prev == first_key;
  const uint32_t a = T.offset[l] + key;
  float* dst = d_params + (size_t)a * 8;
  if (ends && !began_before) {
    reinterpret_cast<float4*>(dst)[0] = make_float4(c[0], c[1], c[2], c[3]);
    reinterpret_cast<float4*>(dst)[1] = make_float4(c[4], c[5], c[6], c[7]);
  } else {
#pragma unroll
    for (int f = 0; f < 8; ++f) atomic_add_f32(dst + f, c[f]);
  }
  if (ends && touched != nullptr && a < q.bitmap_end)
    __hip_atomic_fetch_or(touched + (a >> 5), 1u << (a & 31u), __ATOMIC_RELAXED, __HIP_MEMORY_SCOPE_AGENT);
}

bool dvt_grid_sorted_ok(const DvtGridTable* T, int n);
int dvt_grid_sort_k(const DvtGridTable* T, int k, const float* const* xy, const int32_t* const* ridx, int n, int steps,
                    uint32_t* const* keys, uint16_t* const* pay, float* const* w, hipStream_t s,
                    uint32_t* const* ukeys = nullptr, int32_t* const* ucount = nullptr);
int dvt_grid_gather_k(const DvtGridTable* T, int k, const uint32_t* const* keys, const uint16_t* const* pay,
                      const float* const* w, int n, uint32_t bitmap_end, const float* const* d_enc, float* const* d_params,
                      uint32_t* const* touched, hipStream_t s);

void dvt_grid_bwd_plan(const DvtGridTable& T, int n, GridBwdPlan* plan);
extern int g_grid_lds_chunk;
```

denoising-vit_amd/csrc/dvt_loss_row.h:

```cpp
#pragma once
#include "dvt_common.h"

constexpr int DVT_LOSS_MAXQ = 4;

__device__ __forceinline__ float dvt_sgn(float x) { return (x > 0.f) ? 1.f : ((x < 0.f) ? -1.f : 0.f); }

template <bool HAS_RES>
struct DvtLossRowRegs {
  float4 f[DVT_LOSS_MAXQ], g[DVT_LOSS_MAXQ], r[DVT_LOSS_MAXQ], h[HAS_RES ? DVT_LOSS_MAXQ : 1];
};

template <bool HAS_RES>
__device__ __forceinline__ void dvt_loss_row_load(DvtLossRowRegs<HAS_RES>& x, const float4* __restrict__ F,
                                                  const float4* __restrict__ G, const float4* __restrict__ Hres,
                                                  const float4* __restrict__ raw, int cq, int lane) {
#pragma unroll
  for (int s = 0; s < DVT_LOSS_MAXQ; ++s) {
    const int q = lane + 64 * s;
    if (q < cq) {
      x.f[s] = F[q];
      x.g[s] = G[q];
      x.r[s] = raw[q];
      if (HAS_RES) x.h[s] = Hres[q];
    }
  }
}

template <bool HAS_RES>
__device__ __forceinline__ void dvt_loss_row_compute(const DvtLossRowRegs<HAS_RES>& x, float4* __restrict__ d_pred,
                                                     float4* __restrict__ d_hres, float* __restrict__ d_G,
                                                     float* __restrict__ row_sums, int n, int cq, float grad_scale,
                                                     int lane, uint2* b_pred, uint2* b_hres, float4* f_pred = nullptr,
                                                     float4* f_hres = nullptr) {
  float4 vp[DVT_LOSS_MAXQ], vr[DVT_LOSS_MAXQ], vh[DVT_LOSS_MAXQ], vfg[DVT_LOSS_MAXQ];
  float sse = 0.f, dot = 0.f, np = 0.f, nr = 0.f, rsse = 0.f, rabs = 0.f;
#pragma unroll
  for (int s = 0; s < DVT_LOSS_MAXQ; ++s) {
    const int q = lane + 64 * s;
    if (q < cq) {
      const float4 f = x.f[s], g = x.g[s], r = x.r[s];
      float4 fg = make_float4(f.x + g.x, f.y + g.y, f.z + g.z, f.w + g.w);
      float4 p = fg;
      if (HAS_RES) {
        const float4 h = x.h[s];
        vh[s] = h;
        p = make_float4(fg.x + h.x, fg.y + h.y, fg.z + h.z, fg.w + h.w);
        const float ex = h.x - (r.x - fg.x), ey = h.y - (r.y - fg.y), ez = h.z - (r.z - fg.z),
                    ew = h.w - (r.w - fg.w);
        rsse += ex * ex + ey * ey + ez * ez + ew * ew;
        rabs += fabsf(h.x) + fabsf(h.y) + fabsf(h.z) + fabsf(h.w);
      }
      vp[s] = p;
      vr[s] = r;
      vfg[s] = fg;
      const float dx = p.x - r.x, dy = p.y - r.y, dz = p.z - r.z, dw = p.w - r.w;
      sse += dx * dx + dy * dy + dz * dz + dw * dw;
      dot += p.x * r.x + p.y * r.y + p.z * r.z + p.w * r.w;
      np += p.x * p.x + p.y * p.y + p.z * p.z + p.w * p.w;
      nr += r.x * r.x + r.y * r.y + r.z * r.z + r.w * r.w;
    }
  }
  sse = wave_sum(sse);
  dot = wave_sum(dot);
  np = wave_sum(np);
  nr = wave_sum(nr);
  if (HAS_RES) {
    rsse = wave_sum(rsse);
    rabs = wave_sum(rabs);
  }
  const float n1 = sqrtf(np), n2 = sqrtf(nr);
  const bool clamped = n1 < 1e-8f;
  const float denom = fmaxf(n1, 1e-8f) * fmaxf(n2, 1e-8f);
  const float cosv = dot / denom;
  if (lane == 0 && row_sums != nullptr) {
    row_sums[0] = sse;
    row_sums[1] = cosv;
    row_sums[2] = rsse;
    row_sums[3] = rabs;
  }
  if (d_pred == nullptr && b_pred == nullptr && f_pred == nullptr) return;
  const float inv_nc = 1.0f / ((float)n * (float)(cq * 4));
  const float inv_n = 1.0f / (float)n;
  const float a_r = -inv_n / denom;
  const float a_p = clamped ? 0.f : inv_n * cosv / np;
  const float c_mse = 2.0f * inv_nc;
#pragma unroll
  for (int s = 0; s < DVT_LOSS_MAXQ; ++s) {
    const int q = lane + 64 * s;
    if (q < cq) {
      const float4 p = vp[s], r = vr[s];
      float4 d;
      d.x = grad_scale * (c_mse * (p.x - r.x) + a_r * r.x + a_p * p.x);
      d.y = grad_scale * (c_mse * (p.y - r.y) + a_r * r.y + a_p * p.y);
      d.z = grad_scale * (c_mse * (p.z - r.z) + a_r * r.z + a_p * p.z);
      d.w = grad_scale * (c_mse * (p.w - r.w) + a_r * r.w + a_p * p.w);
      if (d_pred != nullptr) d_pred[q] = d;
      if (b_pred != nullptr) b_pred[q] = make_uint2(dvt_pack_bf16x2(d.x, d.y), dvt_pack_bf16x2(d.z, d.w));
      if (f_pred != nullptr) f_pred[q] = d;
      if (d_G != nullptr) {
        float* g = d_G + q * 4;
        atomic_add_f32(g + 0, d.x);
        atomic_add_f32(g + 1, d.y);
        atomic_add_f32(g + 2, d.z);
        atomic_add_f32(g + 3, d.w);
      }
      if (HAS_RES && (d_hres != nullptr || b_hres != nullptr || f_hres != nullptr)) {
        const float4 h = vh[s], fg = vfg[s];
        const float c_res = 0.1f * 2.0f * inv_nc, c_abs = 0.02f * inv_nc;
        float4 e;
        e.x = grad_scale * (c_res * (h.x - (r.x - fg.x)) + c_abs * dvt_sgn(h.x));
        e.y = grad_scale * (c_res * (h.y - (r.y - fg.y)) + c_abs * dvt_sgn(h.y));
        e.z = grad_scale * (c_res * (h.z - (r.z - fg.z)) + c_abs * dvt_sgn(h.z));
        e.w = grad_scale * (c_res * (h.w - (r.w - fg.w)) + c_abs * dvt_sgn(h.w));
        if (d_hres != nullptr) d_hres[q] = e;
        if (b_hres != nullptr) b_hres[q] = make_uint2(dvt_pack_bf16x2(e.x, e.y), dvt_pack_bf16x2(e.z, e.w));
        if (f_hres != nullptr) f_hres[q] = e;
      }
    }
  }
}

template <bool HAS_RES>
__device__ __forceinline__ void dvt_loss_row(const float4* __restrict__ F, const float4* __restrict__ G,
                                             const float4* __restrict__ Hres, const float4* __restrict__ raw,
                                             float4* __restrict__ d_pred, float4* __restrict__ d_hres,
                                             float* __restrict__ d_G, float* __restrict__ row_sums, int n,
                                             int cq, float grad_scale, int lane, uint2* b_pred, uint2* b_hres) {
  DvtLossRowRegs<HAS_RES> x;
  dvt_loss_row_load<HAS_RES>(x, F, G, Hres, raw, cq, lane);
  dvt_loss_row_compute<HAS_RES>(x, d_pred, d_hres, d_G, row_sums, n, cq, grad_scale, lane, b_pred, b_hres);
}
```

Measured before the change: 2.982.

## Restructure fused row-MLP kernel with cross-layer weight prefetch and early raw loads

```diff
diff --git a/denoising-vit_amd/csrc/dvt_fit_fused.hip b/denoising-vit_amd/csrc/dvt_fit_fused.hip
--- a/denoising-vit_amd/csrc/dvt_fit_fused.hip
+++ b/denoising-vit_amd/csrc/dvt_fit_fused.hip
@@ -8,6 +8,10 @@
 int g_fit_rows32 = 1;
 int g_fit_xcd_affinity = 1;
 int g_fit_small_wg = 0;
+int g_fit_xl_prefetch = 0;
+#ifdef DVT_LAB
+unsigned long long* g_fit_stamps = nullptr;
+#endif
 
 namespace {
 
@@ -30,6 +34,9 @@
   DvtShadowLayout S;
   DvtTLayout TL;
   int n, lattice;
+#ifdef DVT_LAB
+  unsigned long long* stamps;
+#endif
   int xcd_group;
   float grad_scale;
   long long off_grid, off_b1, off_b2, off_G, off_bh1, off_bh2, off_bh3;
@@ -69,90 +76,146 @@
   }
 }
 
-template <int K, int N, bool RELU, bool MASK, int RB, int FW, bool F32>
-__device__ __forceinline__ void mlp_layer(const char* actA, const void* __restrict__ Wv,
-                                          const float* __restrict__ bias, char* act_out,
-                                          float* __restrict__ gout, const char* mask, int wave, int lane) {
-  constexpr int KS = Op<F32>::KS, ES = Op<F32>::ES;
-  constexpr int NTILES = N / 16, NT = (NTILES + FW - 1) / FW, S = K / KS;
-  constexpr int INFL = FW == 8 ? 24 : 16;
-  constexpr int PD0 = INFL / NT > 16 ? 16 : (INFL / NT < 1 ? 1 : INFL / NT);
-  constexpr int PD = PD0 < S ? PD0 : S;
+constexpr int FIT_NSTAMP = 64;
+struct FitStamp {
+#ifdef DVT_LAB
+  unsigned long long* p = nullptr;
+  __device__ __forceinline__ void operator()(int i) const {
+    if (p != nullptr) p[i] = __builtin_amdgcn_s_memrealtime();
+  }
+#else
+  __device__ __forceinline__ void operator()(int) const {}
+#endif
+};
+
+template <int K, int N, int RB, int FW, bool F32>
+struct RowLayer {
+  static constexpr int KS = Op<F32>::KS, ES = Op<F32>::ES;
+  static constexpr int NTILES = N / 16, NT = (NTILES + FW - 1) / FW, S = K / KS;
+  static constexpr int INFL = FW == 8 ? 24 : (FW == 16 ? 12 : 16);
+  static constexpr int PD0 = INFL / NT > 16 ? 16 : (INFL / NT < 1 ? 1 : INFL / NT);
+  static constexpr int PD = PD0 < S ? PD0 : S;
   static_assert(K % KS == 0 && N % 16 == 0, "layer shape");
-  const int lc = lane & 15, g = lane >> 4;
   f32x4 acc[RB][NT];
-  const char* wp[NT];
-#pragma unroll
-  for (int i = 0; i < NT; ++i) {
-#pragma unroll
-    for (int rb = 0; rb < RB; ++rb) acc[rb][i] = (f32x4){0.f, 0.f, 0.f, 0.f};
+  u32x4f b[PD][NT];
+  float bv[NT];
+
+  static __device__ __forceinline__ const char* wptr(const void* __restrict__ Wv, int i, int wave, int lane) {
     const int t = wave + FW * i;
     const int tt = (NTILES % FW == 0 || t < NTILES) ? t : 0;
-    wp[i] = static_cast<const char*>(Wv) + (size_t)tt * S * 1024 + lane * 16;
-  }
-  u32x4f b[PD][NT];
-#pragma unroll
-  for (int p = 0; p < PD; ++p)
-#pragma unroll
-    for (int i = 0; i < NT; ++i) b[p][i] = *reinterpret_cast<const u32x4f*>(wp[i] + 1024 * p);
-  __builtin_amdgcn_sched_barrier(0);
-  const char* ap = actA + lc * apitch<F32>(K) + g * 16;
-#pragma unroll
-  for (int s = 0; s < S; ++s) {
-    u32x4f av[RB];
-#pragma unroll
-    for (int rb = 0; rb < RB; ++rb) av[rb] = *reinterpret_cast<const u32x4f*>(ap + rb * 16 * apitch<F32>(K) + s * 64);
-    if constexpr (F32) {
-#pragma unroll
-      for (int j = 0; j < 4; ++j)
+    return static_cast<const char*>(Wv) + (size_t)tt * S * 1024 + lane * 16;
+  }
+
+  __device__ __forceinline__ void issue(const void* __restrict__ Wv, int wave, int lane) {
+#pragma unroll
+    for (int p = 0; p < PD; ++p)
+#pragma unroll
+      for (int i = 0; i < NT; ++i) b[p][i] = *reinterpret_cast<const u32x4f*>(wptr(Wv, i, wave, lane) + 1024 * p);
+    __builtin_amdgcn_sched_barrier(0);
+  }
+
+  __device__ __forceinline__ void kloop(const char* actA, const void* __restrict__ Wv, int wave, int lane, const FitStamp& st,
+                                        int st0) {
+    const int lc = lane & 15, g = lane >> 4;
+    const char* wp[NT];
+#pragma unroll
+    for (int i = 0; i < NT; ++i) {
+#pragma unroll
+      for (int rb = 0; rb < RB; ++rb) acc[rb][i] = (f32x4){0.f, 0.f, 0.f, 0.f};
+      wp[i] = wptr(Wv, i, wave, lane);
+    }
+    const char* ap = actA + lc * apitch<F32>(K) + g * 16;
+#pragma unroll
+    for (int s = 0; s < S; ++s) {
+      u32x4f av[RB];
+#pragma unroll
+      for (int rb = 0; rb < RB; ++rb) av[rb] = *reinterpret_cast<const u32x4f*>(ap + rb * 16 * apitch<F32>(K) + s * 64);
+      if constexpr (F32) {
+#pragma unroll
+        for (int j = 0; j < 4; ++j)
+#pragma unroll
+          for (int i = 0; i < NT; ++i)
+#pragma unroll
+            for (int rb = 0; rb < RB; ++rb)
+              acc[rb][i] = __builtin_amdgcn_mfma_f32_16x16x4f32(__uint_as_float(av[rb][j]), __uint_as_float(b[s % PD][i][j]),
+                                                                acc[rb][i], 0, 0, 0);
+      } else {
 #pragma unroll
         for (int i = 0; i < NT; ++i)
 #pragma unroll
           for (int rb = 0; rb < RB; ++rb)
-            acc[rb][i] = __builtin_amdgcn_mfma_f32_16x16x4f32(__uint_as_float(av[rb][j]), __uint_as_float(b[s % PD][i][j]),
-                                                              acc[rb][i], 0, 0, 0);
-    } else {
-#pragma unroll
-      for (int i = 0; i < NT; ++i)
-#pragma unroll
-        for (int rb = 0; rb < RB; ++rb)
-          acc[rb][i] = __builtin_amdgcn_mfma_f32_16x16x32_bf16(__builtin_bit_cast(bf16x8, av[rb]),
-                                                               __builtin_bit_cast(bf16x8, b[s % PD][i]), acc[rb][i], 0, 0, 0);
-    }
-    if (s + PD < S) {
-#pragma unroll
-      for (int i = 0; i < NT; ++i) b[s % PD][i] = *reinterpret_cast<const u32x4f*>(wp[i] + 1024 * (s + PD));
-    }
+            acc[rb][i] = __builtin_amdgcn_mfma_f32_16x16x32_bf16(__builtin_bit_cast(bf16x8, av[rb]),
+                                                                 __builtin_bit_cast(bf16x8, b[s % PD][i]), acc[rb][i], 0, 0, 0);
+      }
+      if (s + PD < S) {
+#pragma unroll
+        for (int i = 0; i < NT; ++i) b[s % PD][i] = *reinterpret_cast<const u32x4f*>(wp[i] + 1024 * (s + PD));
+      }
+      if (s == 0) st(st0 + 1);
+      __builtin_amdgcn_sched_barrier(0);
+    }
+  }
+
+  __device__ __forceinline__ void load_bias(const float* __restrict__ bias, int wave, int lane) {
+#pragma unroll
+    for (int i = 0; i < NT; ++i) {
+      const int t = wave + FW * i;
+      bv[i] = (bias != nullptr && (NTILES % FW == 0 || t < NTILES)) ? bias[t * 16 + (lane & 15)] : 0.f;
+    }
+  }
+
+  template <bool RELU, bool MASK>
+  __device__ __forceinline__ void epilogue(char* act_out, float* __restrict__ gout, const char* mask, int wave, int lane) const {
+    const int lc = lane & 15, g = lane >> 4;
+#pragma unroll
+    for (int i = 0; i < NT; ++i) {
+      const int t = wave + FW * i;
+      if (NTILES % FW != 0 && t >= NTILES) continue;
+      const int n = t * 16 + lc;
+#pragma unroll
+      for (int rb = 0; rb < RB; ++rb)
+#pragma unroll
+        for (int r = 0; r < 4; ++r) {
+          const int row = rb * 16 + 4 * g + r;
+          float v = acc[rb][i][r] + bv[i];
+          if (RELU) v = fmaxf(v, 0.f);
+          if (MASK) {
+            if constexpr (F32) {
+              v = *reinterpret_cast<const float*>(mask + row * apitch<F32>(N) + n * ES) > 0.f ? v : 0.f;
+            } else {
+              const uint16_t m = *reinterpret_cast<const uint16_t*>(mask + row * apitch<F32>(N) + n * ES);
+              v = (m != 0 && !(m & 0x8000u)) ? v : 0.f;
+            }
+          }
+          if (act_out != nullptr) {
+            if constexpr (F32) *reinterpret_cast<float*>(act_out + row * apitch<F32>(N) + n * ES) = v;
+            else *reinterpret_cast<uint16_t*>(act_out + row * apitch<F32>(N) + n * ES) = bf16_of(v);
+          }
+          if (gout != nullptr) gout[(size_t)row * N + n] = v;
+        }
+    }
+  }
+};
+struct NoLayer {
+  __device__ __forceinline__ void issue(const void*, int, int) {}
+};
+
+template <bool XL, bool RELU, bool MASK, class LC, class LN>
+__device__ __forceinline__ void run_layer(LC& cur, LN& next, const char* actA, const void* __restrict__ Wcur,
+                                          const void* __restrict__ Wnext, const float* __restrict__ bias, char* act_out,
+                                          float* __restrict__ gout, const char* mask, int wave, int lane, const FitStamp& st,
+                                          int st0) {
+  st(st0);
+  if constexpr (!XL) cur.issue(Wcur, wave, lane);
+  cur.kloop(actA, Wcur, wave, lane, st, st0);
+  st(st0 + 2);
+  cur.load_bias(bias, wave, lane);
+  if constexpr (XL) {
     __builtin_amdgcn_sched_barrier(0);
-  }
-#pragma unroll
-  for (int i = 0; i < NT; ++i) {
-    const int t = wave + FW * i;
-    if (NTILES % FW != 0 && t >= NTILES) continue;
-    const int n = t * 16 + lc;
-    const float bv = bias != nullptr ? bias[n] : 0.f;
-#pragma unroll
-    for (int rb = 0; rb < RB; ++rb)
-#pragma unroll
-      for (int r = 0; r < 4; ++r) {
-        const int row = rb * 16 + 4 * g + r;
-        float v = acc[rb][i][r] + bv;
-        if (RELU) v = fmaxf(v, 0.f);
-        if (MASK) {
-          if constexpr (F32) {
-            v = *reinterpret_cast<const float*>(mask + row * apitch<F32>(N) + n * ES) > 0.f ? v : 0.f;
-          } else {
-            const uint16_t m = *reinterpret_cast<const uint16_t*>(mask + row * apitch<F32>(N) + n * ES);
-            v = (m != 0 && !(m & 0x8000u)) ? v : 0.f;
-          }
-        }
-        if (act_out != nullptr) {
-          if constexpr (F32) *reinterpret_cast<float*>(act_out + row * apitch<F32>(N) + n * ES) = v;
-          else *reinterpret_cast<uint16_t*>(act_out + row * apitch<F32>(N) + n * ES) = bf16_of(v);
-        }
-        if (gout != nullptr) gout[(size_t)row * N + n] = v;
-      }
-  }
+    next.issue(Wnext, wave, lane);
+  }
+  cur.template epilogue<RELU, MASK>(act_out, gout, mask, wave, lane);
+  st(st0 + 3);
 }
 
 template <int C, bool PH2, int FR, bool F32 = false>
@@ -169,14 +232,14 @@
 template <int C>
 constexpr bool fused_f32_fits() { return FusedLds<C, true, 16, true>::TOTAL <= 160 * 1024; }
 
-template <int C, bool PH2, int FR, int FW, bool F32 = false>
+template <int C, bool PH2, int FR, int FW, bool F32 = false, bool XL = false>
 __global__ __launch_bounds__(64 * FW) void fit_rows_kernel(FusedArgs a) {
   using L = FusedLds<C, PH2, FR, F32>;
   constexpr int RB = FR / 16;
   constexpr int ES = Op<F32>::ES;
   static_assert(FR == 16 || FR == 32, "rows per workgroup");
-  static_assert(FW == 8 || (FW == 4 && FR == 16), "waves per workgroup");
-  static_assert(!F32 || (FR == 16 && FW == 8), "fp32 operands: 16 rows, 8 waves");
+  static_assert(FW == 8 || (FW == 4 && FR == 16) || (FW == 16 && FR == 32), "waves per workgroup");
+  static_assert(!F32 || (FR == 16 && FW == 8 && !XL), "fp32 operands: 16 rows, 8 waves, no cross-layer prefetch");
   static_assert(L::TOTAL <= 160 * 1024, "LDS images of the row kernel");
   constexpr int H = C / 2, R = C / 4, E = FE, cq = C / 4;
   __shared__ __attribute__((aligned(16))) char smem[L::TOTAL];
@@ -193,21 +256,32 @@
   const int tid = threadIdx.x, lane = tid & 63;
   const int wave = __builtin_amdgcn_readfirstlane(tid >> 6);
   const int row0 = rb_ * FR;
+  FitStamp st;
+#ifdef DVT_LAB
+  if (a.stamps != nullptr && lane == 0)
+    st.p = a.stamps + ((size_t)((int)blockIdx.x + (int)blockIdx.y * (int)gridDim.x) * FW + wave) * FIT_NSTAMP;
+#endif
+  st(0);
   const char* __restrict__ sh = static_cast<const char*>(f.shadow);
   const float* __restrict__ P = f.params;
   const float4* __restrict__ feat4 = reinterpret_cast<const float4*>(f.feat);
 
-  uint32_t warm[5] = {0u, 0u, 0u, 0u, 0u};
+  DvtGridLevel glev = grid_level(a.T, tid & 15);
+  constexpr int NWP = (FR / FW + 1) / 2, NWW = 32 * RB / FW;
+  uint32_t warm_r[NWP][2], warm_w[NWW];
   {
     constexpr int LPR = (C * 4 + 127) / 128;
-    const int j = lane % 32;
-#pragma unroll
-    for (int rr = lane / 32; rr < FR / FW; rr += 2) {
-      if (j < LPR) {
-        const int ri = f.ridx[row0 + wave + FW * rr];
-        warm[4] ^= __float_as_uint(f.feat[(size_t)ri * C + j * 32]) ^
-                   __float_as_uint(P[a.off_G + (size_t)(ri % a.lattice) * C + j * 32]);
-      }
+    const int j = (lane % 32) < LPR ? lane % 32 : LPR - 1;
+    int ri[NWP];
+#pragma unroll
+    for (int p = 0; p < NWP; ++p) {
+      const int rr = lane / 32 + 2 * p;
+      ri[p] = f.ridx[row0 + wave + FW * (rr < FR / FW ? rr : 0)];
+    }
+#pragma unroll
+    for (int p = 0; p < NWP; ++p) {
+      warm_r[p][0] = __float_as_uint(f.feat[(size_t)ri[p] * C + j * 32]);
+      warm_r[p][1] = __float_as_uint(P[a.off_G + (size_t)(ri[p] % a.lattice) * C + j * 32]);
     }
   }
   {
@@ -219,18 +293,43 @@
     const long long l0 = slot * per, l1 = l0 + per < lines ? l0 + per : lines;
     const uint32_t* w32 = reinterpret_cast<const uint32_t*>(sh);
 #pragma unroll
-    for (int j = 0; j < 4 * RB * (8 / FW); ++j) {
+    for (int j = 0; j < NWW; ++j) {
       const long long li = l0 + tid + (long long)j * 64 * FW;
-      if (li < l1) warm[j & 3] ^= w32[li * 32];
-    }
-  }
-
+      warm_w[j] = w32[(li < l1 ? li : lines - 1) * 32];
+    }
+  }
+  asm volatile("" : "+v"(glev.scale), "+v"(glev.res), "+v"(glev.n), "+v"(glev.off));
+  __builtin_amdgcn_sched_barrier(0);
+
+  constexpr bool RAW_EARLY = PH2 && !F32 && FW >= 8;
+  constexpr int NRAW = RAW_EARLY ? FR * cq / (64 * FW) : 1;
+  static_assert(!RAW_EARLY || (FR * cq) % (64 * FW) == 0, "raw rows: whole float4 rounds of the workgroup");
+  float4 rawv[NRAW];
+  float2 p_enc = make_float2(0.f, 0.f);
+  if constexpr (RAW_EARLY) {
+    const int ri_enc = f.ridx[row0 + (tid < FR * 16 ? tid >> 4 : 0)];
+    __builtin_amdgcn_sched_barrier(0);
+    int ri_raw[NRAW];
+#pragma unroll
+    for (int j = 0; j < NRAW; ++j) ri_raw[j] = f.ridx[row0 + (tid + j * 64 * FW) / cq];
+    __builtin_amdgcn_sched_barrier(0);
+    p_enc = reinterpret_cast<const float2*>(f.xy)[ri_enc];
+    __builtin_amdgcn_sched_barrier(0);
+#pragma unroll
+    for (int j = 0; j < NRAW; ++j) {
+      const int i = tid + j * 64 * FW;
+      rawv[j] = feat4[(size_t)ri_raw[j] * cq + (i - (i / cq) * cq)];
+    }
+    __builtin_amdgcn_sched_barrier(0);
+  }
   if (tid < FR * 16) {
     const int r = tid >> 4, l = tid & 15;
-    const float2 p = reinterpret_cast<const float2*>(f.xy)[f.ridx[row0 + r]];
+    float2 p;
+    if constexpr (RAW_EARLY) p = p_enc;
+    else p = reinterpret_cast<const float2*>(f.xy)[f.ridx[row0 + r]];
     uint32_t idx[4];
     float w[4];
-    corners2d(a.T, l, p.x, p.y, idx, w);
+    corners2d(glev, p.x, p.y, idx, w);
     const float4* __restrict__ grid = reinterpret_cast<const float4*>(P + a.off_grid);
     float4 lo = make_float4(0.f, 0.f, 0.f, 0.f), hi = lo;
 #pragma unroll
@@ -254,7 +353,14 @@
                      dvt_pack_bf16x2(hi.z, hi.w));
     }
   }
-  if (PH2) {
+  if constexpr (RAW_EARLY) {
+#pragma unroll
+    for (int j = 0; j < NRAW; ++j) {
+      const int i = tid + j * 64 * FW, r = i / cq, q = i - r * cq;
+      *reinterpret_cast<uint2*>(smem + L::O_RAW + r * apitch<F32>(C) + q * 8) =
+          make_uint2(dvt_pack_bf16x2(rawv[j].x, rawv[j].y), dvt_pack_bf16x2(rawv[j].z, rawv[j].w));
+    }
+  } else if (PH2) {
     for (int i = tid; i < FR * cq; i += 64 * FW) {
       const int r = i / cq, q = i - r * cq;
       const float4 v = feat4[(size_t)f.ridx[row0 + r] * cq + q];
@@ -265,38 +371,76 @@
             make_uint2(dvt_pack_bf16x2(v.x, v.y), dvt_pack_bf16x2(v.z, v.w));
     }
   }
-  __syncthreads();
-
+  st(1);
   const int B = a.n;
   char* __restrict__ T = static_cast<char*>(f.T);
 #define SH(off) (sh + (size_t)(off) * ES)
 #define TT(idx) (T + (size_t)a.TL.off[idx] * ES)
-  mlp_layer<E, H, true, false, RB, FW, F32>(smem + L::O_ENC, SH(a.S.direct[0]), P + a.off_b1, smem + L::O_H1, nullptr,
-                               nullptr, wave, lane);
-  if (PH2)
-    mlp_layer<C, R, true, false, RB, FW, F32>(smem + L::O_RAW, SH(a.S.direct[2]), P + a.off_bh1, smem + L::O_R1, nullptr,
-                                 nullptr, wave, lane);
+  RowLayer<E, H, RB, FW, F32> lf1;
+  RowLayer<H, C, RB, FW, F32> lf2;
+  RowLayer<C, R, RB, FW, F32> lr1;
+  RowLayer<R, R, RB, FW, F32> lr2;
+  RowLayer<R, C, RB, FW, F32> lr3;
+  RowLayer<C, H, RB, FW, F32> ld1;
+  RowLayer<H, E, RB, FW, F32> ld2;
+  NoLayer none;
+  constexpr bool XLL = XL && FW == 8 && !PH2;
+  {
+    uint32_t warm = 0u;
+#pragma unroll
+    for (int p = 0; p < NWP; ++p) warm ^= warm_r[p][0] ^ warm_r[p][1];
+#pragma unroll
+    for (int j = 0; j < NWW; ++j) warm ^= warm_w[j];
+    asm volatile("" ::"v"(warm));
+  }
+  if constexpr (XL) lf1.issue(SH(a.S.direct[0]), wave, lane);
   __syncthreads();
-  mlp_layer<H, C, false, false, RB, FW, F32>(smem + L::O_H1, SH(a.S.direct[1]), P + a.off_b2, nullptr,
-                                f.F + (size_t)row0 * C, nullptr, wave, lane);
+  st(2);
+  if constexpr (PH2) {
+    run_layer<XL, true, false>(lf1, lr1, smem + L::O_ENC, SH(a.S.direct[0]), SH(a.S.direct[2]), P + a.off_b1, smem + L::O_H1,
+                               nullptr, nullptr, wave, lane, st, 10);
+    run_layer<XL, true, false>(lr1, lf2, smem + L::O_RAW, SH(a.S.direct[2]), SH(a.S.direct[1]), P + a.off_bh1, smem + L::O_R1,
+                               nullptr, nullptr, wave, lane, st, 14);
+  } else {
+    run_layer<XL, true, false>(lf1, lf2, smem + L::O_ENC, SH(a.S.direct[0]), SH(a.S.direct[1]), P + a.off_b1, smem + L::O_H1,
+                               nullptr, nullptr, wave, lane, st, 10);
+  }
+  __syncthreads();
+  st(3);
+  if constexpr (PH2)
+    run_layer<XL, false, false>(lf2, lr2, smem + L::O_H1, SH(a.S.direct[1]), SH(a.S.direct[3]), P + a.off_b2, nullptr,
+                                f.F + (size_t)row0 * C, nullptr, wave, lane, st, 18);
+  else if constexpr (XLL)
+    run_layer<XL, false, false>(lf2, ld1, smem + L::O_H1, SH(a.S.direct[1]), SH(a.S.transp[1]), P + a.off_b2, nullptr,
+                                f.F + (size_t)row0 * C, nullptr, wave, lane, st, 18);
+  else
+    run_layer<XL, false, false>(lf2, none, smem + L::O_H1, SH(a.S.direct[1]), nullptr, P + a.off_b2, nullptr,
+                                f.F + (size_t)row0 * C, nullptr, wave, lane, st, 18);
   store_T<H, FR, FW, F32>(smem + L::O_H1, TT(DVT_T_H1), B, row0, tid);
   store_T<E, FR, FW, F32>(smem + L::O_ENC, TT(DVT_T_ENC), B, row0, tid);
-  if (PH2) {
-    mlp_layer<R, R, true, false, RB, FW, F32>(smem + L::O_R1, SH(a.S.direct[3]), P + a.off_bh2, smem + L::O_R2, nullptr,
-                                 nullptr, wave, lane);
+  if constexpr (PH2) {
+    run_layer<XL, true, false>(lr2, lr3, smem + L::O_R1, SH(a.S.direct[3]), SH(a.S.direct[4]), P + a.off_bh2, smem + L::O_R2,
+                               nullptr, nullptr, wave, lane, st, 22);
     store_T<C, FR, FW, F32>(smem + L::O_RAW, TT(DVT_T_RAW), B, row0, tid);
     store_T<R, FR, FW, F32>(smem + L::O_R1, TT(DVT_T_R1), B, row0, tid);
     __syncthreads();
-    mlp_layer<R, C, false, false, RB, FW, F32>(smem + L::O_R2, SH(a.S.direct[4]), P + a.off_bh3, nullptr,
-                                  f.Hres + (size_t)row0 * C, nullptr, wave, lane);
+    st(4);
+    if constexpr (XLL)
+      run_layer<XL, false, false>(lr3, ld1, smem + L::O_R2, SH(a.S.direct[4]), SH(a.S.transp[1]), P + a.off_bh3, nullptr,
+                                  f.Hres + (size_t)row0 * C, nullptr, wave, lane, st, 26);
+    else
+      run_layer<XL, false, false>(lr3, none, smem + L::O_R2, SH(a.S.direct[4]), nullptr, P + a.off_bh3, nullptr,
+                                  f.Hres + (size_t)row0 * C, nullptr, wave, lane, st, 26);
     store_T<R, FR, FW, F32>(smem + L::O_R2, TT(DVT_T_R2), B, row0, tid);
   }
+  st(5);
   __syncthreads();
+  st(6);
 
   static_assert(C <= 1024, "row warm-up above assumes <= 32 lines per row");
   {
     constexpr int NR = FR / FW;
-    constexpr int NB = (C <= 768 && !(FW == 4 && PH2)) ? 2 : 1;
+    constexpr int NB = (C <= 768 && !(FW == 4 && PH2) && !(FW == 16 && PH2 && C > 384)) ? 2 : 1;
     DvtLossRowRegs<PH2> lr[NB];
 #pragma unroll
     for (int r0 = 0; r0 < NR; r0 += NB) {
@@ -314,7 +458,7 @@
       const int row = wave + FW * rr, gr = row0 + row;
       char* const img_p = smem + L::O_DF + row * apitch<F32>(C);
       char* const img_h = PH2 ? smem + L::O_RAW + row * apitch<F32>(C) : nullptr;
-      dvt_loss_row_compute<PH2>(lr[rr - r0], reinterpret_cast<float4*>(f.dF) + (size_t)gr * cq,
+      dvt_loss_row_compute<PH2, FW == 16>(lr[rr - r0], reinterpret_cast<float4*>(f.dF) + (size_t)gr * cq,
                                 nullptr, nullptr,
                                 f.rows + (size_t)gr * 8, a.n, cq, a.grad_scale, lane,
                                 F32 ? nullptr : reinterpret_cast<uint2*>(img_p), F32 ? nullptr : reinterpret_cast<uint2*>(img_h),
@@ -322,30 +466,42 @@
     }
     }
   }
+  st(7);
+  if constexpr (XL && !XLL) ld1.issue(SH(a.S.transp[1]), wave, lane);
   __syncthreads();
-
-  mlp_layer<C, H, false, true, RB, FW, F32>(smem + L::O_DF, SH(a.S.transp[1]), nullptr, smem + L::O_H1, nullptr,
-                               smem + L::O_H1, wave, lane);
-  store_T<C, FR, FW, F32>(smem + L::O_DF, TT(DVT_T_DF), B, row0, tid);
-  if (PH2) {
-    mlp_layer<C, R, false, true, RB, FW, F32>(smem + L::O_RAW, SH(a.S.transp[4]), nullptr, smem + L::O_R2, nullptr,
-                                 smem + L::O_R2, wave, lane);
+  st(8);
+
+  if constexpr (PH2) {
+    run_layer<XL, false, true>(ld1, lr1, smem + L::O_DF, SH(a.S.transp[1]), SH(a.S.transp[4]), nullptr, smem + L::O_H1, nullptr,
+                               smem + L::O_H1, wave, lane, st, 30);
+    store_T<C, FR, FW, F32>(smem + L::O_DF, TT(DVT_T_DF), B, row0, tid);
+    run_layer<XL, false, true>(lr1, ld2, smem + L::O_RAW, SH(a.S.transp[4]), SH(a.S.transp[0]), nullptr, smem + L::O_R2, nullptr,
+                               smem + L::O_R2, wave, lane, st, 34);
     store_T<C, FR, FW, F32>(smem + L::O_RAW, TT(DVT_T_DH), B, row0, tid);
+  } else {
+    run_layer<XL, false, true>(ld1, ld2, smem + L::O_DF, SH(a.S.transp[1]), SH(a.S.transp[0]), nullptr, smem + L::O_H1, nullptr,
+                               smem + L::O_H1, wave, lane, st, 30);
+    store_T<C, FR, FW, F32>(smem + L::O_DF, TT(DVT_T_DF), B, row0, tid);
   }
   __syncthreads();
-  mlp_layer<H, E, false, false, RB, FW, F32>(smem + L::O_H1, SH(a.S.transp[0]), nullptr, nullptr,
-                                f.denc + (size_t)row0 * E, nullptr, wave, lane);
-  store_T<H, FR, FW, F32>(smem + L::O_H1, TT(DVT_T_DH1), B, row0, tid);
-  if (PH2) {
-    mlp_layer<R, R, false, true, RB, FW, F32>(smem + L::O_R2, SH(a.S.transp[3]), nullptr, smem + L::O_R1, nullptr,
-                                 smem + L::O_R1, wave, lane);
+  st(9);
+  if constexpr (PH2) {
+    run_layer<XL, false, false>(ld2, lr2, smem + L::O_H1, SH(a.S.transp[0]), SH(a.S.transp[3]), nullptr, nullptr,
+                                f.denc + (size_t)row0 * E, nullptr, wave, lane, st, 38);
+    store_T<H, FR, FW, F32>(smem + L::O_H1, TT(DVT_T_DH1), B, row0, tid);
+    run_layer<XL, false, true>(lr2, none, smem + L::O_R2, SH(a.S.transp[3]), nullptr, nullptr, smem + L::O_R1, nullptr,
+                               smem + L::O_R1, wave, lane, st, 42);
     store_T<R, FR, FW, F32>(smem + L::O_R2, TT(DVT_T_DR2), B, row0, tid);
     __syncthreads();
     store_T<R, FR, FW, F32>(smem + L::O_R1, TT(DVT_T_DR1), B, row0, tid);
-  }
+  } else {
+    run_layer<XL, false, false>(ld2, none, smem + L::O_H1, SH(a.S.transp[0]), nullptr, nullptr, nullptr,
+                                f.denc + (size_t)row0 * E, nullptr, wave, lane, st, 38);
+    store_T<H, FR, FW, F32>(smem + L::O_H1, TT(DVT_T_DH1), B, row0, tid);
+  }
+  st(46);
 #undef SH
 #undef TT
-  if (a.n < 0) f.rows[tid] = __uint_as_float(warm[0] ^ warm[1] ^ warm[2] ^ warm[3] ^ warm[4]);
 }
 
 __global__ __launch_bounds__(256) void shadow_build_kernel(DvtShadowLayout L, const float* const p0,
@@ -560,6 +716,17 @@
   wgrad_block<WAVES / 4, F32>(a.w, (int)blockIdx.x, wave, threadIdx.x & 63, smem);
 }
 
+template <int C, int FR, int FW, bool XL>
+void launch_rows_as(const FusedArgs& a, dim3 grid, bool phase2, hipStream_t s) {
+  if (phase2) {
+    if constexpr (FusedLds<C, true, FR>::TOTAL <= 160 * 1024)
+      hipLaunchKernelGGL((fit_rows_kernel<C, true, FR, FW, false, XL>), grid, dim3(64 * FW), 0, s, a);
+  } else {
+    if constexpr (FusedLds<C, false, FR>::TOTAL <= 160 * 1024)
+      hipLaunchKernelGGL((fit_rows_kernel<C, false, FR, FW, false, XL>), grid, dim3(64 * FW), 0, s, a);
+  }
+}
+
 template <int C>
 int launch_rows(const FusedArgs& a, int k, bool phase2, hipStream_t s) {
   if (a.S.f32) {
@@ -574,30 +741,42 @@
   }
   const bool fits32 = phase2 ? (FusedLds<C, true, 32>::TOTAL <= 160 * 1024) : (FusedLds<C, false, 32>::TOTAL <= 160 * 1024);
   const bool r32 = fits32 && a.n % 32 == 0 && (g_fit_rows32 == 2 || (g_fit_rows32 == 1 && k >= 4));
-  const bool small = g_fit_small_wg && !r32;
-  dim3 grid(a.n / (r32 ? 32 : 16), k), block(64 * (small ? 4 : FW8));
+  const bool small = g_fit_small_wg == 1 && !r32;
+  const bool wide = g_fit_small_wg == 2 && r32 && C <= 768;
+  const bool xl = g_fit_xl_prefetch && !small;
+  dim3 grid(a.n / (r32 ? 32 : 16), k);
   FusedArgs ax = a;
   ax.xcd_group = (g_fit_xcd_affinity && (k == 2 || k == 4) && grid.x % (8 / k) == 0 && (grid.x * k) % 8 == 0) ? 8 / k : 0;
-  const FusedArgs& a_ = ax;
-  if (r32) {
-    if (phase2) {
-      if constexpr (FusedLds<C, true, 32>::TOTAL <= 160 * 1024) hipLaunchKernelGGL((fit_rows_kernel<C, true, 32, FW8>), grid, block, 0, s, a_);
-    } else {
-      if constexpr (FusedLds<C, false, 32>::TOTAL <= 160 * 1024) hipLaunchKernelGGL((fit_rows_kernel<C, false, 32, FW8>), grid, block, 0, s, a_);
-    }
+#ifdef DVT_LAB
+  ax.stamps = g_fit_stamps;
+#endif
+  if (wide) {
+    if constexpr (C <= 768) {
+      if (xl) launch_rows_as<C, 32, 16, true>(ax, grid, phase2, s);
+      else launch_rows_as<C, 32, 16, false>(ax, grid, phase2, s);
+    }
+  } else if (r32) {
+    if (xl) launch_rows_as<C, 32, FW8, true>(ax, grid, phase2, s);
+    else launch_rows_as<C, 32, FW8, false>(ax, grid, phase2, s);
   } else if (small) {
-    if (phase2) hipLaunchKernelGGL((fit_rows_kernel<C, true, 16, 4>), grid, block, 0, s, a_);
-    else hipLaunchKernelGGL((fit_rows_kernel<C, false, 16, 4>), grid, block, 0, s, a_);
-  } else if (phase2) {
-    hipLaunchKernelGGL((fit_rows_kernel<C, true, 16, FW8>), grid, block, 0, s, a_);
+    launch_rows_as<C, 16, 4, false>(ax, grid, phase2, s);
+  } else if (xl) {
+    launch_rows_as<C, 16, FW8, true>(ax, grid, phase2, s);
   } else {
-    hipLaunchKernelGGL((fit_rows_kernel<C, false, 16, FW8>), grid, block, 0, s, a_);
+    launch_rows_as<C, 16, FW8, false>(ax, grid, phase2, s);
   }
   DVT_CHECK_LAUNCH();
   return 0;
 }
 
 }
+
+#ifdef DVT_LAB
+extern "C" int dvt_lab_fit_stamps(void* buf) {
+  g_fit_stamps = static_cast<unsigned long long*>(buf);
+  return 0;
+}
+#endif
 
 int dvt_shadow_layout(const DvtFitConfig* c, DvtShadowLayout* L) {
   if (!c || !L) return DVT_E_BADARG;
@@ -766,7 +945,7 @@
   ba.grid_blocks_per_fit = ba.plan.n_lds_blocks + dvt_cdiv(direct_threads, 1024);
   bool sorted = g_fit_sorted_grid && dvt_grid_sorted_ok(&c->grid, c->batch);
   for (int f = 0; f < k; ++f) sorted = sorted && fits[f].gs_keys && fits[f].gs_pay && fits[f].gs_w;
-  const bool small = g_fit_small_wg && sorted && !f32;
+  const bool small = g_fit_small_wg == 1 && sorted && !f32;
   if (sorted) {
     ba.gs.nt = 4 * c->batch;
     ba.gs.bitmap_end = fits[0].gs_bitmap_end;
diff --git a/denoising-vit_amd/csrc/dvt_gemm_f32.hip b/denoising-vit_amd/csrc/dvt_gemm_f32.hip
--- a/denoising-vit_amd/csrc/dvt_gemm_f32.hip
+++ b/denoising-vit_amd/csrc/dvt_gemm_f32.hip
@@ -824,6 +824,7 @@
 extern int g_fit_rows32;
 extern int g_fit_small_wg;
 extern int g_fit_xcd_affinity;
+extern int g_fit_xl_prefetch;
 #ifdef DVT_LAB
 extern int g_fit_skip_mask;
 #endif
@@ -880,7 +881,12 @@
     return 0;
   }
   if (key == 14) {
-    g_fit_small_wg = value != 0;
+    if (value < 0 || value > 2) return DVT_E_BADARG;
+    g_fit_small_wg = value;
+    return 0;
+  }
+  if (key == 17) {
+    g_fit_xl_prefetch = value != 0;
     return 0;
   }
   if (key == 16) {
diff --git a/denoising-vit_amd/csrc/dvt_grid_dev.h b/denoising-vit_amd/csrc/dvt_grid_dev.h
--- a/denoising-vit_amd/csrc/dvt_grid_dev.h
+++ b/denoising-vit_amd/csrc/dvt_grid_dev.h
@@ -1,13 +1,19 @@
 #pragma once
 #include "dvt_common.h"
 
-__device__ __forceinline__ void corners2d(const DvtGridTable& T, int l, float x, float y,
-                                          uint32_t idx[4], float w[4]) {
-  const float scale = T.scale[l];
-  const uint32_t res = T.resolution[l];
-  const uint32_t n = T.entries[l];
-  const uint32_t off = T.offset[l];
-  const bool hashed = T.hashed[l] != 0;
+struct DvtGridLevel {
+  float scale;
+  uint32_t res, n, off;
+  bool hashed;
+};
+__device__ __forceinline__ DvtGridLevel grid_level(const DvtGridTable& T, int l) {
+  return DvtGridLevel{T.scale[l], T.resolution[l], T.entries[l], T.offset[l], T.hashed[l] != 0};
+}
+
+__device__ __forceinline__ void corners2d(const DvtGridLevel& lv, float x, float y, uint32_t idx[4], float w[4]) {
+  const float scale = lv.scale;
+  const uint32_t res = lv.res, n = lv.n, off = lv.off;
+  const bool hashed = lv.hashed;
   const float px = fmaf(scale, x, 0.5f), py = fmaf(scale, y, 0.5f);
   const float fx = floorf(px), fy = floorf(py);
   const uint32_t cx = (uint32_t)(int)fx, cy = (uint32_t)(int)fy;
@@ -22,6 +28,9 @@
     const float b = (c & 2) ? wy : 1.0f - wy;
     w[c] = a * b;
   }
+}
+__device__ __forceinline__ void corners2d(const DvtGridTable& T, int l, float x, float y, uint32_t idx[4], float w[4]) {
+  corners2d(grid_level(T, l), x, y, idx, w);
 }
 
 
diff --git a/denoising-vit_amd/csrc/dvt_loss_row.h b/denoising-vit_amd/csrc/dvt_loss_row.h
--- a/denoising-vit_amd/csrc/dvt_loss_row.h
+++ b/denoising-vit_amd/csrc/dvt_loss_row.h
@@ -26,7 +26,7 @@
   }
 }
 
-template <bool HAS_RES>
+template <bool HAS_RES, bool LEAN = false>
 __device__ __forceinline__ void dvt_loss_row_compute(const DvtLossRowRegs<HAS_RES>& x, float4* __restrict__ d_pred,
                                                      float4* __restrict__ d_hres, float* __restrict__ d_G,
                                                      float* __restrict__ row_sums, int n, int cq, float grad_scale,
@@ -60,6 +60,16 @@
       nr += r.x * r.x + r.y * r.y + r.z * r.z + r.w * r.w;
     }
   }
+  if constexpr (LEAN) {
+#pragma unroll
+    for (int s = 0; s < DVT_LOSS_MAXQ; ++s) {
+      if (lane + 64 * s < cq) {
+        asm volatile("" : "+v"(vr[s].x), "+v"(vr[s].y), "+v"(vr[s].z), "+v"(vr[s].w));
+        asm volatile("" : "+v"(vfg[s].x), "+v"(vfg[s].y), "+v"(vfg[s].z), "+v"(vfg[s].w));
+        if constexpr (HAS_RES) asm volatile("" : "+v"(vh[s].x), "+v"(vh[s].y), "+v"(vh[s].z), "+v"(vh[s].w));
+      }
+    }
+  }
   sse = wave_sum(sse);
   dot = wave_sum(dot);
   np = wave_sum(np);
@@ -88,7 +98,11 @@
   for (int s = 0; s < DVT_LOSS_MAXQ; ++s) {
     const int q = lane + 64 * s;
     if (q < cq) {
-      const float4 p = vp[s], r = vr[s];
+      const float4 r = vr[s];
+      float4 p;
+      if constexpr (!LEAN) p = vp[s];
+      else if constexpr (HAS_RES) p = make_float4(vfg[s].x + vh[s].x, vfg[s].y + vh[s].y, vfg[s].z + vh[s].z, vfg[s].w + vh[s].w);
+      else p = vfg[s];
       float4 d;
       d.x = grad_scale * (c_mse * (p.x - r.x) + a_r * r.x + a_p * p.x);
       d.y = grad_scale * (c_mse * (p.y - r.y) + a_r * r.y + a_p * p.y);
```

Result: no change. 3.000, median of 2 (+0.6%).
